# apple/ml-mdm

Hardware: AMD Instinct MI355X
Metric: denoise-steps/sec, whole job = N x optimizer steps/s at per-GPU batch 64 (train fwd+bwd+optimizer, cc12m_64x64 U-Net) (higher is better)
Workload: dtype bf16; 1 GPU; unet64 train step, per-GPU batch 64, global batch 64; global_batch=64, parallelism=dp1, settle_steps=15

## Files before the change

### include/mdm_hip_ext.h

```cpp
#ifndef MDM_HIP_EXT_H_
#define MDM_HIP_EXT_H_
#ifdef __cplusplus
extern "C" {
#endif

int mdm_attn_cross_bias(const void* qkv, const void* kvc, const float* mask, const float* bias, int bias_ld,
                        const void* base, int base_ld, void* out, int B, int L, int S, int H, int d, int dtype,
                        void* stream);

int mdm_freeu_plan(int N, int H, int W, int C1, int C2, int dtype, int structure, size_t* ws_bytes);
int mdm_freeu_stats(const void* h, const void* r, void* ws, size_t ws_bytes, int N, int H, int W, int C1, int C2,
                    int structure, int dtype, void* stream);
int mdm_freeu_apply(const void* h, const void* r, const void* ws, size_t ws_bytes, void* out, int N, int H, int W, int C1,
                    int C2, float b, float s, int structure, int dtype, void* stream);

int mdm_cfg_plan(int B, size_t chw, int rescale_on, size_t* ws_bytes);
int mdm_cfg_stats(const float* x_t, const float* pred, const float* pred_uncond, const float* gamma, const float* run_prev,
                  float* run_out, const float* run_gate, const float* w_gate, float momentum, int rescale_on, void* ws,
                  size_t ws_bytes, int B, size_t chw, int pred_type, void* stream);
int mdm_cfg_combine(const float* x_t, const float* pred, const float* pred_uncond, const float* gamma, const float* run,
                    const float* w_gate, const void* ws, size_t ws_bytes, float* out, float guidance, float eta,
                    float norm_threshold, float rescale, float image_scale, int B, size_t chw, int pred_type, void* stream);

int mdm_tiles_gather(const float* x, float* out, int B, int C, int H, int W, int h, int w, int sy, int sx, int reps,
                     void* stream);
int mdm_tiles_merge(const float* p, float* out, int R, int C, int H, int W, int h, int w, int sy, int sx, int blend,
                    void* stream);

int mdm_abs_quantile_plan(int B, size_t n, size_t* ws_bytes);
int mdm_abs_quantile(const float* x, void* ws, size_t ws_bytes, int B, size_t n, float q, float cmin, float cmax, float* thr,
                     float* stats, void* stream);

int mdm_t5_attn_fwd_lse(const void* qkv, const int* seq_start, const int* pos, const float* bias_table, void* out, float* lse,
                        int B, int T, int S, int max_len, int H, int d, int dtype, void* stream);
int mdm_t5_attn_bwd(const void* qkv, const void* out, const float* lse, const void* dout, const int* seq_start, const int* pos,
                    const float* bias_table, void* dqkv, int B, int T, int S, int max_len, int H, int d, int dtype,
                    void* stream);
int mdm_t5_gated_gelu_bwd(const void* u, const void* dy, void* du, int T, int F, int dtype, void* stream);
int mdm_t5_rms_bwd(const float* x, const float* ln_w, const void* dh, float* dx, void* dx_lo, int T, int D, float eps,
                   int dtype, void* stream);
int mdm_t5_final_rms_bwd(const float* x, const void* delta, const float* ln_w, const float* dout, const int* flat, float* dx,
                         void* dx_lo, int T, int D, float eps, int dtype, void* stream);
int mdm_t5_embed_rms_slots(const int* ids, const float* table, const int* slot_of_id, const float* learned, const float* ln_w,
                           float* x, void* h, int T, int D, int vocab, int n_ids, int P, float eps, int dtype, void* stream);
int mdm_t5_embed_bwd(const float* dx0, const int* slot_start, const int* tokens, float* dlearned, int P, int D, int n, int T,
                     void* stream);

int mdm_sampler_step_sa(const float* x_t, const float* pred, const float* pred_uncond, float guidance, const float* gamma,
                        const float* gamma_last, const float* gamma_h0, const float* gamma_h1, const float* gate,
                        const float* thr, const float* noise, const unsigned long long* rng_state, int rng_stream, float* h0,
                        float* h1, float* psum, float* x0_out, float* x_last_out, int B, size_t chw, int pred_type, int clip,
                        float image_scale, int max_predictor, int max_corrector, void* stream);

#ifdef __cplusplus
}
#endif
#endif
```

### ml-mdm_amd/csrc/gemm_conv.hip

```cpp
#include <stdio.h>
#include <stdlib.h>

#include <type_traits>
#include <utility>

#include "common.hpp"
#include "conv_args.hpp"

namespace mdm {



__device__ __forceinline__ void load4(const float* p, float (&o)[4]) {
  const f32x4 t = *reinterpret_cast<const f32x4*>(p);
  o[0] = t[0]; o[1] = t[1]; o[2] = t[2]; o[3] = t[3];
}
__device__ __forceinline__ void load4(const bf16* p, float (&o)[4]) {
  const bf16x4 t = *reinterpret_cast<const bf16x4*>(p);
  o[0] = (float)t[0]; o[1] = (float)t[1]; o[2] = (float)t[2]; o[3] = (float)t[3];
}

__device__ __attribute__((aligned(16))) uint4 g_zero_page[4] = {};


// ... 503 lines not shown
#pragma unroll
      for (int i = 0; i < MT; ++i) {
#pragma unroll
        for (int j = 0; j < NT; ++j) mma16(acc[i][j], b0[j], af[i]);
        load_frag<T>(af[i], As, wm * TM + i * 16 + l16, 1, quad);
      }
      __builtin_amdgcn_sched_group_barrier(0x100, NT, 0);
      sched_rows<NT, 0>(std::make_integer_sequence<int, MT>{});
      __builtin_amdgcn_sched_barrier(0);
      asm volatile("s_waitcnt vmcnt(%0)" ::"n"((NSTG - 2) * (AJ + BJ)) : "memory");
      __syncthreads();
      __builtin_amdgcn_sched_barrier(0);
      const char* An = smem + ((kt + 1) % NSTG) * STAGE;
      const char* Bn = An + A_BYTES;
      char* dst = smem + (kt % NSTG) * STAGE;
      MDM_TILE_STATE(kt + NSTG);
#pragma unroll
      for (int j = 0; j < NT; ++j) load_frag<T>(b0[j], Bn, wn * TN + j * 16 + l16, 0, quad);
#pragma unroll
      for (int i = 0; i < MT; ++i) {
#pragma unroll
        for (int j = 0; j < NT; ++j) mma16(acc[i][j], b1[j], af[i]);
#pragma unroll
        for (int d = 0; d < DMA_PER_ROW; ++d) { MDM_DMA_PIECE(dst, i * DMA_PER_ROW + d); }
        load_frag<T>(af[i], An, wm * TM + i * 16 + l16, 0, quad);
      }
      __builtin_amdgcn_sched_group_barrier(0x100, NT, 0);
      sched_rows<NT, DMA_PER_ROW>(std::make_integer_sequence<int, MT>{});
      __builtin_amdgcn_sched_barrier(0);
    }
    asm volatile("s_waitcnt vmcnt(0)" ::: "memory");
    __syncthreads();
    const int cur_m0 = m0, cur_n0 = n0;
    const int next = tile + G;
    if constexpr (SPLITK) {
      float* __restrict__ P = p.part + (size_t)split * p.M * p.Cout;
      if (next < tiles_total) {
        MDM_TILE_SETUP(next);
        MDM_TILE_PROLOGUE();
      }
#pragma unroll
      for (int i = 0; i < MT; ++i) {
        const int m = cur_m0 + wm * TM + i * 16 + l16;
        if (m >= p.M) continue;
#pragma unroll
        for (int j = 0; j < NT; ++j) {
          const int n = cur_n0 + wn * TN + j * 16 + quad * 4;
          if (n < p.Cout) *reinterpret_cast<f32x4*>(P + (size_t)m * p.Cout + n) = acc[i][j];
        }
      }
    } else {
      ConvArgs pe = p;
      if constexpr (GROUPED) { pe.bias = gr.bias[grp]; pe.y = gr.y[grp]; }
      auto prefetch_next = [&]() {
        if (next < tiles_total) {
          MDM_TILE_SETUP(next);
          MDM_TILE_PROLOGUE();
        }
      };
      conv_epilogue<T, BM, BN, WM, WN, NSTG * STAGE, decltype(prefetch_next)>(pe, acc, smem, cur_m0, cur_n0, prefetch_next);
    }
    if (next >= tiles_total) break;
    tile = next;
  }
#undef MDM_TILE_PROLOGUE
#undef MDM_TILE_SETUP
#undef MDM_DMA_PIECE
#undef MDM_TILE_STATE
#undef MDM_BLDS
#endif
}

struct WgradArgs {
  const void* x;
  const void* dy;
  float* slab;
  float* bslab;
  int N, H, W, Cin, Ho, Wo, Cout, stride;
  int M, K;
  int splits, mtiles_per_split;
  int groups;
  int bias_share;
  int skip_cout;
};

constexpr int WG_MAXG = 32;
constexpr int WG_BHDR = 64;
constexpr int WG_BSHARE = 4;
struct WgradGroup {
  const void* x[WG_MAXG];
  const void* dy[WG_MAXG];
  float* out[WG_MAXG];
  float* bout[WG_MAXG];
};

template <typename T, int MODE>
__global__ __launch_bounds__(256) void conv_wgrad_kernel(WgradArgs p) {
  constexpr int EPV = Tr<T>::EPV, BKM = Tr<T>::BK, KSTEPS = Tr<T>::KSTEPS;
  constexpr int BM = 128, BN = 128;
  constexpr int TM = 64, TN = 64, MT = 4, NT = 4;
  constexpr int A_BYTES = BM * 128, STAGE = 2 * A_BYTES;
  constexpr int CPR = 128 / EPV;
  constexpr int MB = BKM / EPV;
  constexpr int BLOCKS = CPR * MB;
  constexpr int NB = 2 * BLOCKS / 256;
  extern __shared__ __attribute__((aligned(16))) char smem[];

  const int tid = threadIdx.x, lane = tid & 63, wave = tid >> 6;
  const int wm = wave >> 1, wn = wave & 1;
  const int quad = lane >> 4, l16 = lane & 15;

  const int tiles_k = (p.K + BN - 1) / BN;
  const int tiles_n = (p.Cout + BM - 1) / BM;
  const int tiles = tiles_k * tiles_n;
  const int lid = xcd_remap(blockIdx.x, gridDim.x);
  const int split = lid / tiles;
  const int t = lid - split * tiles;
  const int n0 = (t / tiles_k) * BM, k0 = (t % tiles_k) * BN;

  const T* __restrict__ X = reinterpret_cast<const T*>(p.x);
  const T* __restrict__ DY = reinterpret_cast<const T*>(p.dy);

  int b_op[NB], b_cc[NB], b_mb[NB];
  int b_tap[NB], b_cin[NB];
  bool b_cvalid[NB];
#pragma unroll
  for (int i = 0; i < NB; ++i) {
    const int id = tid + 256 * i;
    b_op[i] = id / BLOCKS;
    const int r = id - b_op[i] * BLOCKS;
    b_mb[i] = r % MB;
    b_cc[i] = r / MB;
    if (b_op[i] == 0) {
      b_cvalid[i] = (n0 + b_cc[i] * EPV) < p.Cout;
      b_tap[i] = 0; b_cin[i] = 0;
    } else {
      const int k = k0 + b_cc[i] * EPV;
      b_cvalid[i] = k < p.K;
      if (MODE == MODE_1x1) { b_tap[i] = 0; b_cin[i] = k; }
      else { b_tap[i] = k / p.Cin; b_cin[i] = k - b_tap[i] * p.Cin; }
    }
  }

  Blk<T> blk[NB];
  const int mt_begin = split * p.mtiles_per_split;
  const int mt_total = (p.M + BKM - 1) / BKM;
  const int mt_end = min(mt_total, mt_begin + p.mtiles_per_split);

#define MDM_WG_LOAD(mt)                                                                                  \
  {                                                                                                      \
    _Pragma("unroll") for (int i = 0; i < NB; ++i) {                                                     \
      const bool is_a = b_op[i] == 0;                                                                    \
      const T* base = is_a ? DY : X;                                                                     \
      const int mbase = (mt) * BKM + b_mb[i] * EPV;                                                      \
      int pn = 0, poh = 0, pow_ = 0;                                                                     \
      if (MODE != MODE_1x1) {                                                                            \
        const int hw = p.Ho * p.Wo;                                                                      \
        pn = mbase / hw;                                                                                 \
        const int r = mbase - pn * hw;                                                                   \
        poh = r / p.Wo; pow_ = r - poh * p.Wo;                                                           \
      }                                                                                                  \
      const int kh = (b_tap[i] * 11) >> 5, kw = b_tap[i] - 3 * kh;                                       \
      const size_t a_col = (size_t)(n0 + b_cc[i] * EPV);                                                 \
      _Pragma("unroll") for (int e = 0; e < EPV; ++e) {                                                  \
        const int m = mbase + e;                                                                         \
        bool v = b_cvalid[i] && m < p.M;                                                                 \
// ... 543 lines not shown
    for (int c = 0; c < NT; ++c) fb[c] = smem_base + A_BYTES + r0 * ROWB + (((wn * NT + c) ^ fsw) << 5) + ((l16 & 3) << 3);
  }

  if (nt > 0) {
    {
      MDM_WG_TILE_STATE(0);
      MDM_WG_PIECE(smem, 0); MDM_WG_PIECE(smem, 1); MDM_WG_PIECE(smem, 2); MDM_WG_PIECE(smem, 3);
      MDM_WG_PIECE(smem, 4); MDM_WG_PIECE(smem, 5); MDM_WG_PIECE(smem, 6); MDM_WG_PIECE(smem, 7);
    }
    {
      MDM_WG_TILE_STATE(1);
      MDM_WG_PIECE(smem + STAGE, 0); MDM_WG_PIECE(smem + STAGE, 1); MDM_WG_PIECE(smem + STAGE, 2); MDM_WG_PIECE(smem + STAGE, 3);
      MDM_WG_PIECE(smem + STAGE, 4); MDM_WG_PIECE(smem + STAGE, 5); MDM_WG_PIECE(smem + STAGE, 6); MDM_WG_PIECE(smem + STAGE, 7);
    }
    asm volatile("s_waitcnt vmcnt(0)" ::: "memory");
    __syncthreads();
    u32x2 ra[MT][2], rb0[NT][2], rb1[NT][2];
#pragma unroll
    for (int c = 0; c < NT; ++c) MDM_TR2(rb0[c][0], rb0[c][1], fb[c], 0);
#pragma unroll
    for (int c = 0; c < MT; ++c) MDM_TR2(ra[c][0], ra[c][1], fa[c], 0);
    __builtin_amdgcn_sched_barrier(0);

#define MDM_WG_ITER(BIAS)                                                                                   \
    {                                                                                                       \
      const unsigned so = (unsigned)((it & 1) * STAGE), sn = (unsigned)(((it + 1) & 1) * STAGE);            \
                                                                     \
      _Pragma("unroll") for (int c = 0; c < NT; ++c) { const unsigned ad = fb[c] + so; MDM_TR2(rb1[c][0], rb1[c][1], ad, KS1); } \
      Frag<T> bq[NT];                                                                                       \
      _Pragma("unroll") for (int i = 0; i < MT; ++i) {                                                      \
        if (i == 0) {                                                                                       \
          asm volatile("s_waitcnt lgkmcnt(%8)"                                                              \
                       : "+v"(rb0[0][0]), "+v"(rb0[0][1]), "+v"(rb0[1][0]), "+v"(rb0[1][1]), "+v"(rb0[2][0]), \
                         "+v"(rb0[2][1]), "+v"(rb0[3][0]), "+v"(rb0[3][1])                                  \
                       : "n"(WAITN) : "memory");                                                            \
          _Pragma("unroll") for (int j = 0; j < NT; ++j) bq[j] = frag_of(rb0[j][0], rb0[j][1]);             \
        }                                                                                                   \
        asm volatile("s_waitcnt lgkmcnt(%2)" : "+v"(ra[i][0]), "+v"(ra[i][1]) : "n"(WAITN) : "memory");     \
        const Frag<T> aq = frag_of(ra[i][0], ra[i][1]);                                                     \
        _Pragma("unroll") for (int j = 0; j < NT; ++j) mma16(acc[i][j], bq[j], aq);                         \
        if (BIAS && i / BR == wn_s) bsum[i % BR] = frag_sum_guarded(aq, bsum[i % BR]);                      \
        { const unsigned ad = fa[i] + so; MDM_TR2(ra[i][0], ra[i][1], ad, KS1); }                           \
        __builtin_amdgcn_sched_barrier(0);                                                                  \
      }                                                                                                     \
                                        \
      asm volatile("s_waitcnt vmcnt(0) lgkmcnt(0)" ::: "memory");                                           \
      __builtin_amdgcn_s_barrier();                                                                         \
      __builtin_amdgcn_sched_barrier(0);                                                                    \
              \
      MDM_WG_TILE_STATE(it + 2);                                                                            \
      char* const dst = smem + so;                                                                          \
      _Pragma("unroll") for (int c = 0; c < NT; ++c) { const unsigned ad = fb[c] + sn; MDM_TR2(rb0[c][0], rb0[c][1], ad, 0); } \
      _Pragma("unroll") for (int j = 0; j < NT; ++j) bq[j] = frag_of(rb1[j][0], rb1[j][1]);                 \
      _Pragma("unroll") for (int i = 0; i < MT; ++i) {                                                      \
        const Frag<T> aq = frag_of(ra[i][0], ra[i][1]);                                                     \
        _Pragma("unroll") for (int j = 0; j < NT; ++j) mma16(acc[i][j], bq[j], aq);                         \
        if (BIAS && i / BR == wn_s) bsum[i % BR] = frag_sum_guarded(aq, bsum[i % BR]);                      \
        if (MT == 8) { MDM_WG_PIECE_RT(dst, i) } else { MDM_WG_PIECE_RT(dst, 2 * i) MDM_WG_PIECE_RT(dst, 2 * i + 1) } \
        { const unsigned ad = fa[i] + sn; MDM_TR2(ra[i][0], ra[i][1], ad, 0); }                             \
        __builtin_amdgcn_sched_barrier(0);                                                                  \
      }                                                                                                     \
    }
#define MDM_WG_PIECE_RT(stage, q)                                                                           \
    switch (q) {                                                                                            \
      case 0: MDM_WG_PIECE(stage, 0) break; case 1: MDM_WG_PIECE(stage, 1) break;                           \
      case 2: MDM_WG_PIECE(stage, 2) break; case 3: MDM_WG_PIECE(stage, 3) break;                           \
      case 4: MDM_WG_PIECE(stage, 4) break; case 5: MDM_WG_PIECE(stage, 5) break;                           \
      case 6: MDM_WG_PIECE(stage, 6) break; default: MDM_WG_PIECE(stage, 7) break;                          \
    }
    int it = 0;
    float bsum[BR];
    for (; it < bias_b0; ++it) MDM_WG_ITER(false)
#pragma unroll
    for (int i = 0; i < BR; ++i) bsum[i] = 0.f;
    for (; it < bias_b1; ++it) MDM_WG_ITER(true)
    if (bias_blk) {
#pragma unroll
      for (int r = 0; r < BR; ++r) {
        float v = bsum[r];
        v += __shfl_xor(v, 16, 64);
        v += __shfl_xor(v, 32, 64);
        const int n = n0 + wm * TM + (wn * BR + r) * 16 + l16;
        if (quad == 0 && n < p.Cout) {
          if (p.groups > 0) gr.bout[grp][n] += v;
          else p.bslab[((size_t)split * bias_share + kt_rel) * p.Cout + n] = v;
        }
      }
    }
    for (; it < nt; ++it) MDM_WG_ITER(false)
    asm volatile("s_waitcnt vmcnt(0) lgkmcnt(0)" ::: "memory");
#undef MDM_WG_PIECE_RT
#undef MDM_WG_ITER
  } else if (bias_blk && p.groups == 0 && quad == 0) {
#pragma unroll
    for (int r = 0; r < BR; ++r) {
      const int n = n0 + wm * TM + (wn * BR + r) * 16 + l16;
      if (n < p.Cout) p.bslab[((size_t)split * bias_share + kt_rel) * p.Cout + n] = 0.f;
    }
  }
#undef MDM_WG_PIECE
#undef MDM_WG_TILE_STATE
#undef MDM_BLDS

  if (bias_blk && p.groups == 0 && split == 0 && kt_rel == 0 && n0 == 0 && tid == 0)
    reinterpret_cast<int*>(p.bslab - WG_BHDR)[0] = bias_share;
  const bool direct = p.groups > 0;
  float* __restrict__ S = direct ? gr.out[grp] : p.slab + (size_t)split * p.Cout * p.K;
  const bool vec_ok = (p.K & 3) == 0;
  if (!direct) {
#pragma unroll
    for (int i = 0; i < MT; ++i) {
      const int n = n0 + wm * TM + i * 16 + l16;
      if (n >= p.Cout) continue;
#pragma unroll
      for (int j = 0; j < NT; ++j) {
        const int k = k0 + wn * TN + j * 16 + quad * 4;
        if (k >= p.K) continue;
        float* o = S + (size_t)n * p.K + k;
        if (vec_ok) {
          *reinterpret_cast<f32x4*>(o) = acc[i][j];
        } else {
#pragma unroll
          for (int e = 0; e < 4; ++e) if (k + e < p.K) o[e] = acc[i][j][e];
        }
      }
    }
  } else if (vec_ok && n0 + BM <= p.Cout && k0 + BN <= p.K) {
    float* const o0 = S + (size_t)(n0 + wm * TM + l16) * p.K + k0 + wn * TN + quad * 4;
    f32x4 old[2][NT];
#pragma unroll
    for (int j = 0; j < NT; ++j) old[0][j] = *reinterpret_cast<const f32x4*>(o0 + j * 16);
#pragma unroll
    for (int i = 0; i < MT; ++i) {
      if (i + 1 < MT) {
#pragma unroll
        for (int j = 0; j < NT; ++j) old[(i + 1) & 1][j] = *reinterpret_cast<const f32x4*>(o0 + (size_t)(i + 1) * 16 * p.K + j * 16);
      }
#pragma unroll
      for (int j = 0; j < NT; ++j) *reinterpret_cast<f32x4*>(o0 + (size_t)i * 16 * p.K + j * 16) = old[i & 1][j] + acc[i][j];
    }
  } else {
#pragma unroll
    for (int i = 0; i < MT; ++i) {
      const int n = n0 + wm * TM + i * 16 + l16;
      if (n >= p.Cout) continue;
#pragma unroll
      for (int j = 0; j < NT; ++j) {
        const int k = k0 + wn * TN + j * 16 + quad * 4;
        if (k >= p.K) continue;
        float* o = S + (size_t)n * p.K + k;
#pragma unroll
        for (int e = 0; e < 4; ++e) if (k + e < p.K) o[e] += acc[i][j][e];
      }
    }
  }
#endif
}
#undef MDM_TR2

template <int NT>
__device__ __forceinline__ void wgrad_bias_reduce(const float* __restrict__ bslab, float* __restrict__ dbias, int splits,
                                                  int Cout, int accumulate, int blk, float* lds) {
  constexpr int G = NT / 32;
  const int tid = threadIdx.x, c = tid & 31, g = tid >> 5;
  const int rows = splits * reinterpret_cast<const int*>(bslab - WG_BHDR)[0];
  const int o = blk * 32 + c;
  float s0 = 0.f, s1 = 0.f, s2 = 0.f, s3 = 0.f;
  if (o < Cout) {
    const float* src = bslab + o;
    int r = g;
    for (; r + 3 * G < rows; r += 4 * G) {
      s0 += src[(size_t)r * Cout];
      s1 += src[(size_t)(r + G) * Cout];
      s2 += src[(size_t)(r + 2 * G) * Cout];
      s3 += src[(size_t)(r + 3 * G) * Cout];
    }
    for (; r < rows; r += G) s0 += src[(size_t)r * Cout];
  }
  lds[tid] = (s0 + s1) + (s2 + s3);
  __syncthreads();
  if (g == 0 && o < Cout) {
    float s = lds[c];
#pragma unroll
    for (int q = 1; q < G; ++q) s += lds[q * 32 + c];
    dbias[o] = accumulate ? dbias[o] + s : s;
  }
}

__global__ __launch_bounds__(192) void wgrad_reduce_kernel(const float* __restrict__ slab, float* __restrict__ dw,
                                                           const float* __restrict__ bslab, float* __restrict__ dbias,
                                                           int splits, int Cout, int Cin, int taps, int accumulate,
                                                           int bblocks) {
// ... 1122 lines not shown
  a.mtiles_per_split = (mt_total + a.splits - 1) / a.splits;
  float* const bias_ws = ws + (size_t)a.splits * Cout * a.K;
  a.bslab = (want_bias && dtype == DT_BF16) ? bias_ws + WG_BHDR : nullptr;
  const int te = wgrad_tile(a.M, Cout, a.K, dtype);
  const int tiles = ((Cout + te - 1) / te) * ((a.K + te - 1) / te);
  {
    const int kt = skip_cout > 0 ? Cin / te : (a.K + te - 1) / te;
    a.bias_share = kt < WG_BSHARE ? (kt < 1 ? 1 : kt) : WG_BSHARE;
  }
  hipStream_t st = reinterpret_cast<hipStream_t>(stream);
  if (wgrad_direct_slabs(a.M, Cout, a.K, dtype) && wgrad_direct_ok(a, ksize)) {
    return launch_wgrad_direct<64, 9, 8>(a, st);
  }
  constexpr int smem = 4 * 128 * 128, smem_big = 4 * 64 * 512;
  ensure_dynamic_lds(conv_wgrad_kernel<float, MODE_1x1>, smem);
  ensure_dynamic_lds(conv_wgrad_kernel<float, MODE_3x3>, smem);
  ensure_dynamic_lds(conv_wgrad_tr_kernel<MODE_1x1, 0>, smem);
  ensure_dynamic_lds(conv_wgrad_tr_kernel<MODE_3x3, 0>, smem);
  ensure_dynamic_lds(conv_wgrad_tr_kernel<MODE_1x1, 1>, smem_big);
  ensure_dynamic_lds(conv_wgrad_tr_kernel<MODE_3x3, 1>, smem_big);
  ensure_dynamic_lds(conv_wgrad_bl_kernel<MODE_1x1, 0>, smem);
  ensure_dynamic_lds(conv_wgrad_bl_kernel<MODE_3x3, 0>, smem);
  ensure_dynamic_lds(conv_wgrad_bl_kernel<MODE_1x1, 1>, smem_big);
  ensure_dynamic_lds(conv_wgrad_bl_kernel<MODE_3x3, 1>, smem_big);
  dim3 grid(tiles * a.splits);
  const int mode = ksize == 1 ? MODE_1x1 : MODE_3x3;
  if (dtype == DT_F32) MDM_NOTE_KERNEL("conv_wgrad_kernel<float, %d>", mode);
  else if (wgrad_bl_ok(a, ksize)) MDM_NOTE_KERNEL("conv_wgrad_bl_kernel<%d, %d>", mode, te == 256 ? 1 : 0);
  else MDM_NOTE_KERNEL("conv_wgrad_tr_kernel<%d, %d>", mode, te == 256 ? 1 : 0);
  if (dtype == DT_F32) {
    if (ksize == 1) hipLaunchKernelGGL((conv_wgrad_kernel<float, MODE_1x1>), grid, dim3(256), smem, st, a);
    else hipLaunchKernelGGL((conv_wgrad_kernel<float, MODE_3x3>), grid, dim3(256), smem, st, a);
  } else if (wgrad_bl_ok(a, ksize)) {
    if (te == 256) {
      if (ksize == 1) hipLaunchKernelGGL((conv_wgrad_bl_kernel<MODE_1x1, 1>), grid, dim3(512), smem_big, st, a, WgradGroup{});
      else hipLaunchKernelGGL((conv_wgrad_bl_kernel<MODE_3x3, 1>), grid, dim3(512), smem_big, st, a, WgradGroup{});
    } else {
      if (ksize == 1) hipLaunchKernelGGL((conv_wgrad_bl_kernel<MODE_1x1, 0>), grid, dim3(256), smem, st, a, WgradGroup{});
      else hipLaunchKernelGGL((conv_wgrad_bl_kernel<MODE_3x3, 0>), grid, dim3(256), smem, st, a, WgradGroup{});
    }
  } else if (te == 256) {
    if (ksize == 1) hipLaunchKernelGGL((conv_wgrad_tr_kernel<MODE_1x1, 1>), grid, dim3(512), smem_big, st, a);
    else hipLaunchKernelGGL((conv_wgrad_tr_kernel<MODE_3x3, 1>), grid, dim3(512), smem_big, st, a);
  } else {
    if (ksize == 1) hipLaunchKernelGGL((conv_wgrad_tr_kernel<MODE_1x1, 0>), grid, dim3(256), smem, st, a);
    else hipLaunchKernelGGL((conv_wgrad_tr_kernel<MODE_3x3, 0>), grid, dim3(256), smem, st, a);
  }
  MDM_LAUNCH_STATUS();
}

extern "C" int mdm_conv_wgrad(const void* x, const void* dy, int want_bias, float* ws, int N, int H, int W, int Cin,
                              int Ho, int Wo, int Cout, int ksize, int stride, int dtype, void* stream) {
  return conv_wgrad_impl(x, dy, want_bias, ws, N, H, W, Cin, Ho, Wo, Cout, ksize, stride, dtype, 0, stream);
}

extern "C" int mdm_conv_wgrad_blocked(const void* x, const void* dyb, int want_bias, float* ws, int N, int H, int W, int Cin,
                                      int Cout, int dtype, void* stream) {
  MDM_CHECK_ARG(dtype == DT_BF16 && Cin % 256 == 0 && Cout % 256 == 0);
  MDM_CHECK_ARG((H & (H - 1)) == 0 && (W & (W - 1)) == 0);
  return conv_wgrad_impl(x, dyb, want_bias, ws, N, H, W, Cin, H, W, 4 * Cout, 3, 1, dtype, Cout, stream);
}

static int wgrad_group_tile(int M, int Cout, int K, int groups) {
  if (groups < 2 || groups > WG_MAXG || M < 4096) return 0;
  if (const int forced = wgrad_forced_tile(Cout, K, DT_BF16)) return forced;
  const long t256 = (long)((Cout + 255) / 256) * ((K + 255) / 256) * groups;
  const long t128 = (long)((Cout + 127) / 128) * ((K + 127) / 128) * groups;
  const int cus = device_cus();
  if (Cout >= 192 && K >= 192) {
    const double eff = (double)t256 / (double)(((t256 + cus - 1) / cus) * cus);
    if (t256 >= (long)(0.7 * cus) && eff >= 0.7) return 256;
  }
  const double eff = (double)t128 / (double)(((t128 + 2 * cus - 1) / (2 * cus)) * 2 * cus);
  if (t128 >= (long)(1.4 * cus) && eff >= 0.7) return 128;
  return 0;
}

extern "C" int mdm_conv_wgrad_group_plan(int M, int Cout, int K, int dtype, int groups, int* tile_out) {
  MDM_CHECK_ARG(tile_out);
  *tile_out = dtype == DT_BF16 ? wgrad_group_tile(M, Cout, K, groups) : 0;
  return 0;
}

extern "C" int mdm_conv_wgrad_grouped(const void* const* x, const void* const* dy, float* const* dw,
                                      float* const* dbias, int groups, int M, int Cin, int Cout, int dtype,
                                      void* stream) {
  MDM_CHECK_ARG(x && dy && dw && groups >= 1 && groups <= WG_MAXG);
  MDM_CHECK_ARG(dtype == DT_BF16 && Cin % 8 == 0 && Cout % 8 == 0 && M > 0);
  WgradArgs a = {};
  a.N = M; a.H = 1; a.W = 1; a.Cin = Cin; a.Ho = 1; a.Wo = 1; a.Cout = Cout; a.stride = 1;
  a.M = M; a.K = Cin; a.splits = 1; a.groups = groups;
  a.mtiles_per_split = (M + 63) / 64;
  MDM_CHECK_ARG(wgrad_bl_ok(a, 1));
  WgradGroup gr = {};
  for (int g = 0; g < groups; ++g) {
    MDM_CHECK_ARG(x[g] && dy[g] && dw[g]);
    gr.x[g] = x[g]; gr.dy[g] = dy[g]; gr.out[g] = dw[g]; gr.bout[g] = dbias ? dbias[g] : nullptr;
  }
  int te = wgrad_group_tile(M, Cout, Cin, groups);
  if (!te) te = wgrad_forced_tile(Cout, Cin, DT_BF16);
  if (!te) te = (Cout >= 192 && Cin >= 192) ? 256 : 128;
  const int tiles = ((Cout + te - 1) / te) * ((Cin + te - 1) / te);
  hipStream_t st = reinterpret_cast<hipStream_t>(stream);
  constexpr int smem = 4 * 128 * 128, smem_big = 4 * 64 * 512;
  if (te == 256) {
    ensure_dynamic_lds(conv_wgrad_bl_kernel<MODE_1x1, 1>, smem_big);
    hipLaunchKernelGGL((conv_wgrad_bl_kernel<MODE_1x1, 1>), dim3(tiles * groups), dim3(512), smem_big, st, a, gr);
  } else {
    ensure_dynamic_lds(conv_wgrad_bl_kernel<MODE_1x1, 0>, smem);
    hipLaunchKernelGGL((conv_wgrad_bl_kernel<MODE_1x1, 0>), dim3(tiles * groups), dim3(256), smem, st, a, gr);
  }
  MDM_NOTE_KERNEL("conv_wgrad_bl_kernel<%d, %d>", MODE_1x1, te == 256 ? 1 : 0);
  MDM_LAUNCH_STATUS();
}

extern "C" int mdm_conv_wgrad_reduce(const float* ws, float* dw_oihw, float* dbias, const void* dy, int M, int Cin,
                                     int Cout, int ksize, int accumulate, int dtype, void* stream) {
  MDM_CHECK_ARG(ws && dw_oihw && (ksize == 1 || ksize == 3));
  const int K = ksize * ksize * Cin;
  int splits; size_t wsb;
  int rc = mdm_conv_wgrad_plan(M, Cout, K, dtype, &splits, &wsb);
  if (rc) return rc;
  hipStream_t st = reinterpret_cast<hipStream_t>(stream);
  float* const bias_ws = const_cast<float*>(ws) + (size_t)splits * Cout * K;
  const float* bslab = (dbias && dtype == DT_BF16) ? bias_ws + WG_BHDR : nullptr;
  const int bblocks = bslab ? (Cout + 31) / 32 : 0;
  if (ksize == 1) {
    const size_t total = (size_t)Cout * Cin;
    const int wblocks = (int)((total / 4 + 255) / 256 > 2048 ? 2048 : (total / 4 + 255) / 256);
    hipLaunchKernelGGL(wgrad_reduce_flat_kernel, dim3(wblocks + bblocks), dim3(256), 0, st, ws, dw_oihw, bslab, dbias,
                       splits, Cout, total, accumulate, wblocks, bblocks);
  } else {
    const int wblocks = Cout * ((Cin + 63) / 64);
    hipLaunchKernelGGL(wgrad_reduce_kernel, dim3(wblocks + bblocks), dim3(192), 0, st, ws, dw_oihw, bslab, dbias,
                       splits, Cout, Cin, ksize * ksize, accumulate, bblocks);
  }
  if (dbias && !bslab) {
    MDM_CHECK_ARG(dy);
    return mdm_colsum(dy, dbias, bias_ws, M, Cout, accumulate, dtype, stream);
  }
  MDM_LAUNCH_STATUS();
}

extern "C" int mdm_pack_weight(const float* w_oihw, void* w_fwd, void* w_dgrad, int Cout, int Cin, int ksize,
                               int Cin_pad, int Cout_pad, int kblock_fwd, int kblock_dgrad, int dtype,
                               void* stream) {
  MDM_CHECK_ARG(w_oihw && w_fwd);
  MDM_CHECK_ARG(ksize == 1 || ksize == 3);
  MDM_CHECK_ARG(Cin_pad >= Cin && Cout_pad >= Cout);
  MDM_CHECK_ARG(kblock_fwd == 0 || (ksize == 3 && Cin_pad % kblock_fwd == 0));
  MDM_CHECK_ARG(kblock_dgrad == 0 || (ksize == 3 && Cout_pad % kblock_dgrad == 0));
  const int taps = ksize * ksize;
  const size_t total = (size_t)Cout * taps * Cin_pad + (w_dgrad ? (size_t)Cin * taps * Cout_pad : 0);
  const int nb = (int)((total + 255) / 256 > 8192 ? 8192 : (total + 255) / 256);
  hipStream_t st = reinterpret_cast<hipStream_t>(stream);
  if (Cin_pad == Cin && Cout_pad == Cout && Cin % 32 == 0 && Cout % 32 == 0) {
    dim3 grid(Cin / 32, Cout / 32);
#define MDM_PACK_TILED(TT, TAPS)                                                                               \
  hipLaunchKernelGGL((pack_weight_tiled_kernel<TT, TAPS>), grid, dim3(256), 0, st, w_oihw, (TT*)w_fwd, (TT*)w_dgrad, \
                     Cout, Cin, kblock_fwd, kblock_dgrad)
    if (dtype == DT_F32) { if (taps == 9) MDM_PACK_TILED(float, 9); else MDM_PACK_TILED(float, 1); }
    else if (dtype == DT_BF16) { if (taps == 9) MDM_PACK_TILED(bf16, 9); else MDM_PACK_TILED(bf16, 1); }
    else MDM_CHECK_ARG(false);
#undef MDM_PACK_TILED
    MDM_LAUNCH_STATUS();
  }
  if (dtype == DT_F32)
    hipLaunchKernelGGL(pack_weight_kernel<float>, dim3(nb), dim3(256), 0, st, w_oihw, (float*)w_fwd, (float*)w_dgrad, Cout, Cin, taps, Cin_pad, Cout_pad, kblock_fwd, kblock_dgrad);
  else if (dtype == DT_BF16)
    hipLaunchKernelGGL(pack_weight_kernel<bf16>, dim3(nb), dim3(256), 0, st, w_oihw, (bf16*)w_fwd, (bf16*)w_dgrad, Cout, Cin, taps, Cin_pad, Cout_pad, kblock_fwd, kblock_dgrad);
  else MDM_CHECK_ARG(false);
  MDM_LAUNCH_STATUS();
}

extern "C" int mdm_pack_weights_multi(const void* table, int n, int total_blocks, int dtype, void* stream) {
  MDM_CHECK_ARG(table && n > 0 && total_blocks > 0);
  static_assert(sizeof(PackDesc) == 48, "descriptor layout is part of the ABI");
  hipStream_t st = reinterpret_cast<hipStream_t>(stream);
  if (dtype == DT_F32) hipLaunchKernelGGL(pack_weights_multi_kernel<float>, dim3(total_blocks), dim3(256), 0, st, (const PackDesc*)table, n);
  else if (dtype == DT_BF16) hipLaunchKernelGGL(pack_weights_multi_kernel<bf16>, dim3(total_blocks), dim3(256), 0, st, (const PackDesc*)table, n);
  else MDM_CHECK_ARG(false);
  MDM_LAUNCH_STATUS();
}

static inline int colsum_slabs(int M, int C, int epv) {
  const int groups = (C + 8 * epv - 1) / (8 * epv);
  int slabs = (1024 + groups - 1) / groups;
  const int max_slabs = (M + 63) / 64;
  if (slabs > max_slabs) slabs = max_slabs;
  if (slabs > 64) slabs = 64;
  if (slabs < 1) slabs = 1;
  return slabs;
}

extern "C" int mdm_colsum_plan(int M, int C, int* nblocks, size_t* ws_bytes) {
  MDM_CHECK_ARG(nblocks && ws_bytes);
// ... 24 lines not shown
```

### ml-mdm_amd/csrc/norm.hip

```cpp
#include <stdlib.h>

#include "common.hpp"

namespace mdm {

template <int N> struct GnInt { static constexpr int value = N; };

template <int ACT>
__device__ __forceinline__ float gn_affine_act(float a, float x, float b) {
  const float z = a * x + b;
  return ACT ? silu_f(z) : z;
}


template <typename T>
__global__ __launch_bounds__(256) void gn_partial_kernel(const T* __restrict__ x, float* __restrict__ part,
                                                         int HW, int C, int slabs, int pix_per_slab) {
  constexpr int EPV = Tr<T>::EPV;
  __shared__ float red[256 * 16];
  const int n = blockIdx.x / slabs, slab = blockIdx.x - n * slabs;
  const int tid = threadIdx.x;
  const int nchunks = C / EPV;
  const int p_begin = slab * pix_per_slab, p_end = min(HW, p_begin + pix_per_slab);
  const T* xn = x + (size_t)n * HW * C;
// ... 1006 lines not shown
#define MDM_GN_REAPPLY(TT, ACT, DROP)                                                                                \
  hipLaunchKernelGGL((gn_reapply_kernel<TT, ACT, DROP>), grid, dim3(256), 0, st, (const TT*)x, coef, (TT*)y, HW, C, lanes, \
                     ppb, thresh, scale, seed, offset)
#define MDM_GN_REAPPLY_T(TT)                                                                                         \
  if (p > 0.f) { if (act) MDM_GN_REAPPLY(TT, 1, true); else MDM_GN_REAPPLY(TT, 0, true); }                           \
  else { if (act) MDM_GN_REAPPLY(TT, 1, false); else MDM_GN_REAPPLY(TT, 0, false); }
  if (dtype == DT_F32) { MDM_GN_REAPPLY_T(float) } else { MDM_GN_REAPPLY_T(bf16) }
#undef MDM_GN_REAPPLY_T
#undef MDM_GN_REAPPLY
  MDM_LAUNCH_STATUS();
}

extern "C" int mdm_gn_bwd(const void* dy, const void* x, const float* gamma, const float* beta, const void* film,
                          const float* stats, const float* coef, const void* dres, const void* dres2, void* dx,
                          float* dgamma, float* dbeta, void* dfilm, float* ws, int N, int HW, int C, int G, int act,
                          int accumulate, int dtype, void* stream) {
  MDM_CHECK_ARG(dy && x && gamma && beta && stats && coef && dx && dgamma && dbeta && ws);
  MDM_CHECK_ARG(dtype == DT_F32 || dtype == DT_BF16);
  MDM_CHECK_ARG((film == nullptr) == (dfilm == nullptr));
  if (!dres && dres2) { dres = dres2; dres2 = nullptr; }
  const int epv = dtype == DT_F32 ? 4 : 8;
  MDM_CHECK_ARG(C % epv == 0 && C % G == 0 && C <= 2048 && G <= 256);
  hipStream_t st = reinterpret_cast<hipStream_t>(stream);
  MDM_CHECK_ARG(accumulate >= 0 && accumulate <= 2);
  const int pstride = accumulate == 2 ? C : 0;
  if (!accumulate) {
    if (hipMemsetAsync(dgamma, 0, (size_t)C * sizeof(float), st) != hipSuccess ||
        hipMemsetAsync(dbeta, 0, (size_t)C * sizeof(float), st) != hipSuccess) {
      mdm_set_error(__FILE__, __LINE__, "hipMemsetAsync(dgamma / dbeta)");
      return (int)hipGetLastError();
    }
  }
  if (const GnFusedCfg f = gn_fused_cfg(HW, C, G, dtype, true); f.cb) {
    const dim3 grid(N, C / f.cb);
    const int cb = f.cb;
#define MDM_GN_FUSED_BWD_L(TT, ACT, NI_, NT_, LPR_)                                                                 \
    hipLaunchKernelGGL((gn_fused_bwd_kernel<TT, ACT, NI_, NT_, LPR_>), grid, dim3(NT_), 0, st, (const TT*)dy, (const TT*)x, gamma, beta, (const TT*)film, stats, coef, (TT*)dx, (TT*)dfilm, dgamma, dbeta, (const TT*)dres, (const TT*)dres2, HW, C, G, cb, pstride)
#define MDM_GN_FUSED_BWD(TT, ACT, LPR_)                                                                             \
    if (f.nthr == 512 && f.ni == 4) MDM_GN_FUSED_BWD_L(TT, ACT, 4, 512, LPR_);                                     \
    else if (f.nthr == 512) MDM_GN_FUSED_BWD_L(TT, ACT, 16, 512, LPR_);                                            \
    else MDM_GN_FUSED_BWD_L(TT, ACT, 4, 1024, LPR_)
    if (dtype == DT_F32) { if (act) { MDM_GN_FUSED_BWD(float, 1, 16); } else { MDM_GN_FUSED_BWD(float, 0, 16); } }
    else { if (act) { MDM_GN_FUSED_BWD(bf16, 1, 8); } else { MDM_GN_FUSED_BWD(bf16, 0, 8); } }
#undef MDM_GN_FUSED_BWD
#undef MDM_GN_FUSED_BWD_L
    MDM_LAUNCH_STATUS();
  }
  const int cb = gn_slice(C, G, epv);
  MDM_CHECK_ARG(cb > 0);
  const size_t esize = dtype == DT_F32 ? 4 : 2;
  int nchunk = 1;
  while (nchunk < 8 && N % (nchunk * 2) == 0 && N / (nchunk * 2) >= 4 &&
         2 * (size_t)N * HW * C * esize / nchunk > g_gn_chunk_bytes)
    nchunk *= 2;
  if ((size_t)(N / nchunk) * gn_slabs(N / nchunk, HW) > (size_t)N * gn_slabs(N, HW)) nchunk = 1;
  const int nc = N / nchunk;
  const int slabs = gn_slabs(nc, HW);
  const int pps = (HW + slabs - 1) / slabs;
  const int sp = gn_pix_splits(nc, HW, C / cb);
  const int ppb = (HW + sp - 1) / sp;
  const dim3 agrid(sp, C / cb, nc);
#define MDM_GN_BWD(TT, ACT)                                                                                          \
  for (int ch = 0; ch < nchunk; ++ch) {                                                                              \
    const size_t n0 = (size_t)ch * nc, t0 = n0 * HW * C;                                                             \
    const TT* film_ = film ? (const TT*)film + n0 * 2 * C : nullptr;                                                 \
    TT* dfilm_ = dfilm ? (TT*)dfilm + n0 * 2 * C : nullptr;                                                          \
    const TT* dres_ = dres ? (const TT*)dres + t0 : nullptr;                                                         \
    const TT* dres2_ = dres2 ? (const TT*)dres2 + t0 : nullptr;                                                      \
    hipLaunchKernelGGL((gn_bwd_partial_kernel<TT, ACT>), dim3(nc * slabs), dim3(256), 0, st, (const TT*)dy + t0,     \
                       (const TT*)x + t0, coef + n0 * C * 2, ws, HW, C, slabs, pps);                                 \
    hipLaunchKernelGGL((gn_bwd_apply_kernel<TT, ACT>), agrid, dim3(256), 0, st, (const TT*)dy + t0, (const TT*)x + t0, ws, \
                       stats + n0 * G * 2, coef + n0 * C * 2, gamma, beta, film_, dres_, dres2_, (TT*)dx + t0, dfilm_, \
                       dgamma + n0 * pstride, dbeta + n0 * pstride, HW, C, G, cb, slabs, ppb, pstride);              \
  }
  if (dtype == DT_F32) { if (act) { MDM_GN_BWD(float, 1) } else { MDM_GN_BWD(float, 0) } }
  else { if (act) { MDM_GN_BWD(bf16, 1) } else { MDM_GN_BWD(bf16, 0) } }
#undef MDM_GN_BWD
  MDM_LAUNCH_STATUS();
}

struct GnParamDesc {
  const float* pg; const float* pb;
  float* dgamma; float* dbeta;
  int N, C, first_block, pad_;
};

__global__ __launch_bounds__(256) void gn_param_reduce_multi_kernel(const GnParamDesc* __restrict__ table, int n) {
  __shared__ float red[2][4][64];
  const int lb = (int)blockIdx.x >> 2, sub = (int)blockIdx.x & 3;
  int lo = 0, hi = n - 1;
  while (lo < hi) {
    const int mid = (lo + hi + 1) >> 1;
    if (table[mid].first_block <= lb) lo = mid; else hi = mid - 1;
  }
  const GnParamDesc d = table[lo];
  const int cl = (int)threadIdx.x & 63, q = (int)threadIdx.x >> 6;
  const int c = (lb - d.first_block) * 256 + sub * 64 + cl;
  float a = 0.f, b = 0.f;
  if (c < d.C) {
    int s_ = q;
    for (; s_ + 12 < d.N; s_ += 16) {
      const float a0 = d.pg[(size_t)s_ * d.C + c], a1 = d.pg[(size_t)(s_ + 4) * d.C + c];
      const float a2 = d.pg[(size_t)(s_ + 8) * d.C + c], a3 = d.pg[(size_t)(s_ + 12) * d.C + c];
      const float b0 = d.pb[(size_t)s_ * d.C + c], b1 = d.pb[(size_t)(s_ + 4) * d.C + c];
      const float b2 = d.pb[(size_t)(s_ + 8) * d.C + c], b3 = d.pb[(size_t)(s_ + 12) * d.C + c];
      a += (a0 + a1) + (a2 + a3);
      b += (b0 + b1) + (b2 + b3);
    }
    for (; s_ < d.N; s_ += 4) { a += d.pg[(size_t)s_ * d.C + c]; b += d.pb[(size_t)s_ * d.C + c]; }
  }
  red[0][q][cl] = a; red[1][q][cl] = b;
  __syncthreads();
  if (q == 0 && c < d.C) {
    d.dgamma[c] += (red[0][0][cl] + red[0][1][cl]) + (red[0][2][cl] + red[0][3][cl]);
    d.dbeta[c] += (red[1][0][cl] + red[1][1][cl]) + (red[1][2][cl] + red[1][3][cl]);
  }
}

extern "C" int mdm_gn_param_reduce_multi(const void* table, int n, int total_blocks, void* stream) {
  MDM_CHECK_ARG(table && n > 0 && total_blocks > 0);
  static_assert(sizeof(GnParamDesc) == 48, "descriptor layout is part of the ABI");
  hipLaunchKernelGGL(gn_param_reduce_multi_kernel, dim3(4 * total_blocks), dim3(256), 0, reinterpret_cast<hipStream_t>(stream),
                     (const GnParamDesc*)table, n);
  MDM_LAUNCH_STATUS();
}

extern "C" int mdm_ln_fwd(const void* x, const float* gamma, const float* beta, void* y, float* stats, int R, int D,
                          float eps, int dtype, void* stream) {
  MDM_CHECK_ARG(x && gamma && beta && y && stats && R > 0 && D > 0);
  hipStream_t st = reinterpret_cast<hipStream_t>(stream);
  if (dtype == DT_F32) hipLaunchKernelGGL(ln_fwd_kernel<float>, dim3(R), dim3(256), 0, st, (const float*)x, gamma, beta, (float*)y, stats, D, eps);
  else if (dtype == DT_BF16) hipLaunchKernelGGL(ln_fwd_kernel<bf16>, dim3(R), dim3(256), 0, st, (const bf16*)x, gamma, beta, (bf16*)y, stats, D, eps);
  else MDM_CHECK_ARG(false);
  MDM_LAUNCH_STATUS();
}

extern "C" int mdm_ln_bwd(const void* dy, const void* x, const float* gamma, const float* stats, void* dx,
                          float* dgamma, float* dbeta, float* ws, int R, int D, int accumulate, int dtype,
                          void* stream) {
  MDM_CHECK_ARG(dy && x && gamma && stats && dx && dgamma && dbeta && ws);
  hipStream_t st = reinterpret_cast<hipStream_t>(stream);
  const int rpb = 64, nsl = (R + rpb - 1) / rpb;
  if (dtype == DT_F32) {
    hipLaunchKernelGGL(ln_bwd_kernel<float>, dim3(R), dim3(256), 0, st, (const float*)dy, (const float*)x, gamma, stats, (float*)dx, D);
    hipLaunchKernelGGL(ln_bwd_param_partial_kernel<float>, dim3((D + 255) / 256, nsl), dim3(256), 0, st, (const float*)dy, (const float*)x, stats, ws, R, D, rpb);
  } else if (dtype == DT_BF16) {
    hipLaunchKernelGGL(ln_bwd_kernel<bf16>, dim3(R), dim3(256), 0, st, (const bf16*)dy, (const bf16*)x, gamma, stats, (bf16*)dx, D);
    hipLaunchKernelGGL(ln_bwd_param_partial_kernel<bf16>, dim3((D + 255) / 256, nsl), dim3(256), 0, st, (const bf16*)dy, (const bf16*)x, stats, ws, R, D, rpb);
  } else MDM_CHECK_ARG(false);
  hipLaunchKernelGGL(ln_bwd_param_final_kernel, dim3((D + 255) / 256), dim3(256), 0, st, ws, dgamma, dbeta, nsl, D, accumulate);
  MDM_LAUNCH_STATUS();
}

extern "C" int mdm_ln_multi_fwd(const void* x, const float* const* gamma, const float* const* beta, void* const* y, int L,
                                float* stats, int R, int D, float eps, int dtype, void* stream) {
  MDM_CHECK_ARG(x && gamma && beta && y && stats && L >= 1 && L <= LN_MAXL && R > 0 && D > 0);
  MDM_CHECK_ARG(dtype == DT_F32 ? (D % 4 == 0 && D <= 256 * 4 * LN_NCK) : (D % 8 == 0 && D <= 256 * 8 * LN_NCK));
  LnGroup g = {};
  for (int l = 0; l < L; ++l) { MDM_CHECK_ARG(gamma[l] && beta[l] && y[l]); g.gamma[l] = gamma[l]; g.beta[l] = beta[l]; g.y[l] = y[l]; }
  hipStream_t st = reinterpret_cast<hipStream_t>(stream);
  if (dtype == DT_F32) hipLaunchKernelGGL(ln_multi_fwd_kernel<float>, dim3(R), dim3(256), 0, st, (const float*)x, g, L, stats, D, eps);
  else if (dtype == DT_BF16) hipLaunchKernelGGL(ln_multi_fwd_kernel<bf16>, dim3(R), dim3(256), 0, st, (const bf16*)x, g, L, stats, D, eps);
  else MDM_CHECK_ARG(false);
  MDM_LAUNCH_STATUS();
}

extern "C" int mdm_ln_multi_bwd(const void* const* dy, const void* x, const float* const* gamma, const float* stats,
                                void* dx, float* const* dgamma, float* const* dbeta, int L, int R, int D, int accumulate,
                                int dtype, void* stream) {
  MDM_CHECK_ARG(dy && x && gamma && stats && dx && dgamma && dbeta && L >= 1 && L <= LN_MAXL && R > 0 && D > 0 && D <= 4096);
  MDM_CHECK_ARG(D % (dtype == DT_F32 ? 4 : 8) == 0);
  LnGroup g = {};
  hipStream_t st = reinterpret_cast<hipStream_t>(stream);
  for (int l = 0; l < L; ++l) {
    MDM_CHECK_ARG(dy[l] && gamma[l] && dgamma[l] && dbeta[l]);
    g.y[l] = const_cast<void*>(dy[l]); g.gamma[l] = gamma[l]; g.dgamma[l] = dgamma[l]; g.dbeta[l] = dbeta[l];
    if (!accumulate) {
      (void)hipMemsetAsync(dgamma[l], 0, (size_t)D * sizeof(float), st);
      (void)hipMemsetAsync(dbeta[l], 0, (size_t)D * sizeof(float), st);
    }
  }
  const int rpb = 64, nsl = (R + rpb - 1) / rpb;
  if (dtype == DT_F32) {
    hipLaunchKernelGGL(ln_multi_bwd_kernel<float>, dim3(R), dim3(256), 0, st, g, L, (const float*)x, stats, (float*)dx, D);
    hipLaunchKernelGGL(ln_multi_param_kernel<float>, dim3((D + 255) / 256, nsl, L), dim3(256), 0, st, g, (const float*)x, stats, R, D, rpb);
  } else if (dtype == DT_BF16) {
    hipLaunchKernelGGL(ln_multi_bwd_kernel<bf16>, dim3(R), dim3(256), 0, st, g, L, (const bf16*)x, stats, (bf16*)dx, D);
    hipLaunchKernelGGL(ln_multi_param_kernel<bf16>, dim3((D + 255) / 256, nsl, L), dim3(256), 0, st, g, (const bf16*)x, stats, R, D, rpb);
  } else MDM_CHECK_ARG(false);
  MDM_LAUNCH_STATUS();
}
```

### ml-mdm_amd/csrc/optim.hip

```cpp
#include "common.hpp"

namespace mdm {

__global__ __launch_bounds__(256) void sumsq_partial_kernel(const float* __restrict__ g, float* __restrict__ part,
                                                            size_t n4) {
  __shared__ float sh[4];
  float s = 0.f;
  const f32x4* g4 = reinterpret_cast<const f32x4*>(g);
  for (size_t i = (size_t)blockIdx.x * 256 + threadIdx.x; i < n4; i += (size_t)gridDim.x * 256) {
    const f32x4 v = g4[i];
    s += v[0] * v[0] + v[1] * v[1] + v[2] * v[2] + v[3] * v[3];
  }
  s = wave_sum(s);
  if ((threadIdx.x & 63) == 0) sh[threadIdx.x >> 6] = s;
  __syncthreads();
  if (threadIdx.x == 0) part[blockIdx.x] = sh[0] + sh[1] + sh[2] + sh[3];
}

__global__ __launch_bounds__(256) void sumsq_final_kernel(const float* __restrict__ part, int nparts,
                                                          const float* __restrict__ g, size_t n, size_t tail_from,
                                                          float* __restrict__ out, int* __restrict__ step_counter) {
  __shared__ float sh[4];
  float s = 0.f;
  for (int i = threadIdx.x; i < nparts; i += 256) s += part[i];
  for (size_t i = tail_from + threadIdx.x; i < n; i += 256) s += g[i] * g[i];
  s = wave_sum(s);
  if ((threadIdx.x & 63) == 0) sh[threadIdx.x >> 6] = s;
  __syncthreads();
  if (threadIdx.x == 0) {
    const float q = sh[0] + sh[1] + sh[2] + sh[3];
    out[0] = q;
    if (step_counter && q == q && q <= 3.0e38f) step_counter[0] += 1;
  }
}

struct AdamArgs {
  float* p; float* g; float* m; float* v; float* ema;
  const float* gnorm_sq;
  const int* step_dev;
  size_t n;
  float lr, beta1, beta2, eps, wd, bc1, bc2, clip, ema_decay;
  int zero_grad;
};

__device__ __forceinline__ void adam_one(float& p, float& g, float& m, float& v, float& e, const AdamArgs& a, float gs,
                                         bool has_ema) {
  const float gr = g * gs;
  p *= (1.f - a.lr * a.wd);
  m = a.beta1 * m + (1.f - a.beta1) * gr;
  v = a.beta2 * v + (1.f - a.beta2) * gr * gr;
  const float denom = sqrtf(v) / sqrtf(a.bc2) + a.eps;
  p -= (a.lr / a.bc1) * (m / denom);
  if (has_ema) e = e * a.ema_decay + p * (1.f - a.ema_decay);
  if (a.zero_grad) g = 0.f;
}

__global__ __launch_bounds__(256) void adamw_ema_kernel(AdamArgs a) {
  if (a.step_dev) {
    const float st = (float)a.step_dev[0];
    a.bc1 = 1.f - powf(a.beta1, st);
    a.bc2 = 1.f - powf(a.beta2, st);
  }
  float gs = 1.f;
  bool poisoned = false;
  if (a.gnorm_sq) {
    const float q = a.gnorm_sq[0];
    poisoned = !(q == q) || q > 3.0e38f;
    const float nrm = sqrtf(q);
    gs = fminf(a.clip / (nrm + 1e-6f), 1.f);
  }
  const bool has_ema = a.ema != nullptr;
  const size_t n4 = a.n / 4;
  f32x4* p4 = reinterpret_cast<f32x4*>(a.p);
  f32x4* g4 = reinterpret_cast<f32x4*>(a.g);
  if (poisoned) {
    if (a.zero_grad) {
      for (size_t i = (size_t)blockIdx.x * 256 + threadIdx.x; i < n4; i += (size_t)gridDim.x * 256) g4[i] = f32x4{0.f, 0.f, 0.f, 0.f};
      if (blockIdx.x == 0) for (size_t i = n4 * 4 + threadIdx.x; i < a.n; i += 256) a.g[i] = 0.f;
    }
    return;
  }
  f32x4* m4 = reinterpret_cast<f32x4*>(a.m);
  f32x4* v4 = reinterpret_cast<f32x4*>(a.v);
  f32x4* e4 = reinterpret_cast<f32x4*>(a.ema);
  for (size_t i = (size_t)blockIdx.x * 256 + threadIdx.x; i < n4; i += (size_t)gridDim.x * 256) {
    f32x4 p = p4[i], g = g4[i], m = m4[i], v = v4[i];
    f32x4 e = has_ema ? e4[i] : f32x4{0.f, 0.f, 0.f, 0.f};
#pragma unroll
    for (int k = 0; k < 4; ++k) {
      float pp = p[k], gg = g[k], mm = m[k], vv = v[k], ee = e[k];
      adam_one(pp, gg, mm, vv, ee, a, gs, has_ema);
      p[k] = pp; g[k] = gg; m[k] = mm; v[k] = vv; e[k] = ee;
    }
    p4[i] = p; m4[i] = m; v4[i] = v;
    if (has_ema) e4[i] = e;
    if (a.zero_grad) g4[i] = g;
  }
  if (blockIdx.x == 0) {
    for (size_t i = n4 * 4 + threadIdx.x; i < a.n; i += 256) {
      float e = has_ema ? a.ema[i] : 0.f;
      adam_one(a.p[i], a.g[i], a.m[i], a.v[i], e, a, gs, has_ema);
      if (has_ema) a.ema[i] = e;
    }
  }
}

}

using namespace mdm;

extern "C" int mdm_sumsq(const float* g, float* out, float* ws, size_t n, int* step_counter, void* stream) {
  MDM_CHECK_ARG(g && out && ws);
  MDM_CHECK_ARG(((size_t)g & 15) == 0);
  hipStream_t st = reinterpret_cast<hipStream_t>(stream);
  const size_t n4 = n / 4;
  int nb = (int)((n4 + 255) / 256 > 1024 ? 1024 : (n4 + 255) / 256);
  if (nb < 1) nb = 1;
  hipLaunchKernelGGL(sumsq_partial_kernel, dim3(nb), dim3(256), 0, st, g, ws, n4);
  hipLaunchKernelGGL(sumsq_final_kernel, dim3(1), dim3(256), 0, st, ws, nb, g, n, n4 * 4, out, step_counter);
  MDM_LAUNCH_STATUS();
}

extern "C" int mdm_adamw_ema_step(float* p, float* g, float* m, float* v, float* ema, const float* gnorm_sq, size_t n,
                                  float lr, float beta1, float beta2, float eps, float weight_decay, int step,
                                  const int* step_dev, float clip, float ema_decay, int zero_grad, void* stream) {
  MDM_CHECK_ARG(p && g && m && v && (step >= 1 || step_dev));
  MDM_CHECK_ARG((((size_t)p | (size_t)g | (size_t)m | (size_t)v | (size_t)ema) & 15) == 0);
  AdamArgs a;
  a.p = p; a.g = g; a.m = m; a.v = v; a.ema = ema; a.gnorm_sq = gnorm_sq; a.n = n;
  a.lr = lr; a.beta1 = beta1; a.beta2 = beta2; a.eps = eps; a.wd = weight_decay;
  a.step_dev = step_dev;
  a.bc1 = 1.f - powf(beta1, (float)(step >= 1 ? step : 1));
  a.bc2 = 1.f - powf(beta2, (float)(step >= 1 ? step : 1));
  a.clip = clip; a.ema_decay = ema_decay; a.zero_grad = zero_grad;
  hipStream_t st = reinterpret_cast<hipStream_t>(stream);
  const size_t n4 = n / 4;
  int nb = (int)((n4 + 255) / 256 > 8192 ? 8192 : (n4 + 255) / 256);
  if (nb < 1) nb = 1;
  hipLaunchKernelGGL(adamw_ema_kernel, dim3(nb), dim3(256), 0, st, a);
  MDM_LAUNCH_STATUS();
}
```

### ml-mdm_amd/mdm_hip/distributed.py

```python
import os
from datetime import timedelta

import torch
import torch.distributed as dist


def get_rank() -> int:
    return dist.get_rank() if dist.is_available() and dist.is_initialized() else 0


def get_world_size() -> int:
    return dist.get_world_size() if dist.is_available() and dist.is_initialized() else 1


def get_local_rank() -> int:
    return int(os.environ.get("LOCAL_RANK", "0"))


def print0(*a, **k):
    if get_rank() == 0:
        print(*a, **k)


def init_distributed_singlenode(timeout: int = 0, backend: str = None):
    world = int(os.environ.get("WORLD_SIZE", "1"))
    if world == 1 or "MASTER_ADDR" not in os.environ:
        return get_local_rank(), int(os.environ.get("RANK", "0")), 1
    rank, local = int(os.environ["RANK"]), get_local_rank()
    if backend is None:
        backend = "nccl" if torch.cuda.is_available() else "gloo"
    kw = {"timeout": timedelta(seconds=timeout)} if timeout else {}
    if backend == "nccl":
        torch.cuda.set_device(local)
    dist.init_process_group(backend=backend, init_method="env://", world_size=world, rank=rank, **kw)
    barrier(local)
    return local, rank, world


def barrier(local_rank: int = None):
    if dist.get_backend() == "nccl":
        dist.barrier(device_ids=[torch.cuda.current_device() if local_rank is None else local_rank])
    else:
        dist.barrier()


class GradReducer:

    def __init__(self, params, bucket_mb: float = 256.0, wire_dtype="auto", group=None, tail_mb: float = 8.0,
                 world_override: int = None, force_collectives: bool = False, head_mb: float = 64.0,
                 record_timeline: bool = False, late_params=None):
        self.params = [p for p in params if p.requires_grad]
        self.group = group
        self.nranks = dist.get_world_size(group) if dist.is_initialized() else 1
        if world_override is not None:
            self.nranks = int(world_override)
        self.world = self.nranks if not (force_collectives and self.nranks == 1 and dist.is_initialized()) else 2
        self._wire_auto = False
        if isinstance(wire_dtype, str):
            if wire_dtype != "auto":
                raise ValueError("wire_dtype: a torch dtype, None (fp32) or 'auto'")
            wire_dtype = None
        self.wire_dtype = wire_dtype
        self._wire = {}
        self._comm = None
        self._avg_ok = None
        self.record_timeline = bool(record_timeline)
        self._timeline = []
        self._t0 = None
        dev = self.params[0].device
        total = sum(p.numel() for p in self.params)
        self.flat = torch.zeros(total, dtype=torch.float32, device=dev)
        order = list(reversed(self.params))
        late = {id(p) for p in (late_params or [])}
        if late:
            order = [p for p in order if id(p) not in late] + [p for p in order if id(p) in late]
        self.order = order
        cap = max(1, int(bucket_mb * (1 << 20) / 4))
        tail = min(int(tail_mb * (1 << 20) / 4), cap)
        head = max(1, min(int(head_mb * (1 << 20) / 4), cap)) if head_mb else cap
        tail_from, acc = len(order), 0
        for i in range(len(order) - 1, -1, -1):
            acc += order[i].numel()
            if acc > tail:
                break
            tail_from = i
        self.buckets = []
        self._bucket_of = {}
        off = b_start = 0
        for i, p in enumerate(order):
            if i == tail_from and off > b_start:
                self.buckets.append((b_start, off))
                b_start = off
            n = p.numel()
            p.grad = self.flat[off:off + n].view_as(p)
            self._bucket_of[p] = len(self.buckets)
            off += n
            if off - b_start >= (head if not self.buckets else cap):
                self.buckets.append((b_start, off))
                b_start = off
        if off > b_start:
            self.buckets.append((b_start, off))
        self._slots = {p.data_ptr(): (p, p.grad) for p in self.params}
        self._grad_ptrs = [(p, p.grad.data_ptr()) for p in self.params]
        self._need = [0] * len(self.buckets)
        for p in order:
            self._need[self._bucket_of[p]] += 1
        self._pending = list(self._need)
        self._fired = {}
        self._deferred = set()
        self._streams = [set() for _ in self.buckets]
        self._work = []
        self._enabled = True
        if self.world > 1:
            for p in self.params:
                p.register_post_accumulate_grad_hook(self._hook)

    def slot(self, p):
        ent = self._slots.get(p.data_ptr())
        return ent[1] if ent is not None and ent[0].shape == p.shape else None

    def ready(self, p):
        if self.world > 1:
            self._count(self._slots[p.data_ptr()][0])

    def defer(self, p):
        if self.world > 1:
            self._deferred.add(id(self._slots[p.data_ptr()][0]))

    def rebind(self):
        self._slots = {p.data_ptr(): (p, p.grad) for p in self.params}

    def _hook(self, p):
        if id(p) in self._deferred:
            return
        self._count(p)

    def note_autocast(self, bf16: bool):
        return None

    def _comm_stream(self):
        if self._comm is None:
            self._comm = torch.cuda.Stream(device=self.flat.device)
        return self._comm

    def _post_stream(self):
        if getattr(self, "_post", None) is None:
            self._post = torch.cuda.Stream(device=self.flat.device)
        return self._post

    def _count(self, p):
        if not self._enabled:
            return
        b = self._bucket_of[p]
        if id(p) in self._fired:
            return
        self._fired[id(p)] = 1
        if p.is_cuda:
            self._streams[b].add(torch.cuda.current_stream())
        self._pending[b] -= 1
        if self._pending[b] == 0:
            self._launch(b)

    def _launch(self, b):
        s, e = self.buckets[b]
        buf = self.flat[s:e]
        if not buf.is_cuda:
            buf.div_(self.nranks)
            if self.wire_dtype is not None and self.wire_dtype != torch.float32:
                wire = buf.to(self.wire_dtype)
                h = dist.all_reduce(wire, op=dist.ReduceOp.SUM, group=self.group, async_op=True)
                self._work.append((h, buf, wire, None))
            else:
                h = dist.all_reduce(buf, op=dist.ReduceOp.SUM, group=self.group, async_op=True)
                self._work.append((h, None, None, None))
            return
        comm = self._comm_stream()
        for st in self._streams[b]:
            ev = torch.cuda.Event()
            ev.record(st)
            comm.wait_event(ev)
        self._streams[b] = set()
        post = self._post_stream()
        with torch.cuda.stream(comm):
            ev0 = None
            if self.record_timeline:
                if self._t0 is None:
                    self._t0 = torch.cuda.Event(enable_timing=True)
                    self._t0.record(comm)
                ev0 = torch.cuda.Event(enable_timing=True)
                ev0.record(comm)
            scale = 1.0 / self.nranks
            if self.wire_dtype is not None and self.wire_dtype != torch.float32:
                wire = self._wire.get(b)
                if wire is None:
                    wire = self._wire[b] = torch.empty(e - s, dtype=self.wire_dtype, device=buf.device)
                if self.nranks > 1:
                    torch.mul(buf, scale, out=wire)
                else:
                    wire.copy_(buf)
                h = dist.all_reduce(wire, op=dist.ReduceOp.SUM, group=self.group, async_op=True)
                nbytes = wire.numel() * wire.element_size()
            else:
                wire = None
                if self._avg_ok is None:
                    self._avg_ok = dist.get_backend(self.group) == "nccl" and hasattr(dist.ReduceOp, "AVG")
                if self._avg_ok and self.nranks > 1:
                    h = dist.all_reduce(buf, op=dist.ReduceOp.AVG, group=self.group, async_op=True)
                else:
                    if self.nranks > 1:
                        buf.mul_(scale)
                    h = dist.all_reduce(buf, op=dist.ReduceOp.SUM, group=self.group, async_op=True)
                nbytes = buf.numel() * 4
        with torch.cuda.stream(post):
            h.wait()
            if wire is not None:
                buf.copy_(wire)
            done = None
            if ev0 is not None:
                done = torch.cuda.Event(enable_timing=True)
                done.record(post)
                self._timeline.append([b, nbytes, ev0, done])
        self._work.append((h, None, None, ev0))

    def no_sync(self):
        reducer = self

        class _Ctx:
            def __enter__(self):
                reducer._enabled = False

            def __exit__(self, *a):
                reducer._enabled = True

        return _Ctx()

    def check_bound(self):
        for p, ptr in self._grad_ptrs:
            if p.grad is None or p.grad.data_ptr() != ptr:
                raise RuntimeError("a parameter's .grad no longer points into the GradReducer arena (zero_grad(set_to_none=True)?); "
                                   "use GradReducer.zero_grad()")

    def finish(self):
        self.check_bound()
        if self.world > 1 and self._enabled:
            if self._pending == self._need and not self._work:
                self._deferred = set()
                return
            missing = [b for b, n in enumerate(self._pending) if n != 0]
            if missing:
                lost = [(i, tuple(p.shape), self._fired.get(id(p), 0)) for i, p in enumerate(self.params) if self._fired.get(id(p), 0) != 1]
                raise RuntimeError("buckets %s did not receive all their gradients; parameters (index, shape) that "
                                   "did not report exactly once (index, shape, count): %s" % (missing, lost[:12]))
            if self._comm is not None and self.flat.is_cuda:
                torch.cuda.current_stream().wait_stream(self._post_stream())
            else:
                for h, buf, wire, _ in self._work:
                    h.wait()
                    if wire is not None:
                        buf.copy_(wire)
            self._work = []
            if self.record_timeline:
                self._last_timeline, self._last_t0 = self._timeline, self._t0
                self._timeline, self._t0 = [], None
            self._pending = list(self._need)
            self._fired = {}
        self._deferred = set()

    def mark(self, what):
        if self.record_timeline and self.flat.is_cuda and self.world > 1:
            ev = torch.cuda.Event(enable_timing=True)
            ev.record()
            setattr(self, "_" + what, ev)

    def backward_window_ms(self):
        b0, b1, t0 = getattr(self, "_bw0", None), getattr(self, "_bw1", None), getattr(self, "_last_t0", None)
        if b0 is None or b1 is None or t0 is None:
            return None
        torch.cuda.synchronize()
        return b0.elapsed_time(t0), b0.elapsed_time(b1)

    def timeline(self):
        tl, t0 = getattr(self, "_last_timeline", None), getattr(self, "_last_t0", None)
        if not tl or t0 is None:
            return []
        torch.cuda.synchronize()
        return [(b, nb, t0.elapsed_time(e0), t0.elapsed_time(e1) if e1 is not None else float("nan")) for b, nb, e0, e1 in tl]

    def zero_grad(self):
        self.flat.zero_()

    def broadcast_parameters(self, src: int = 0):
        if self.nranks == 1:
            return
        with torch.no_grad():
            chunk, acc = [], 0
            for p in self.params:
                chunk.append(p)
                acc += p.numel()
                if acc * 4 >= (256 << 20):
                    self._bcast(chunk, src)
                    chunk, acc = [], 0
            if chunk:
                self._bcast(chunk, src)

    def _bcast(self, ps, src):
        flat = torch.cat([p.detach().reshape(-1) for p in ps])
        dist.broadcast(flat, src, group=self.group)
        off = 0
        for p in ps:
            p.copy_(flat[off:off + p.numel()].view_as(p))
            off += p.numel()


class DataParallel(torch.nn.Module):

    _IGNORED = {"output_device", "dim", "broadcast_buffers", "process_group", "bucket_cap_mb", "check_reduction",
                "gradient_as_bucket_view", "init_sync", "device_mesh", "mixed_precision", "delay_all_reduce_named_params",
                "param_to_hook_all_reduce"}
    _UNSUPPORTED = {"find_unused_parameters", "static_graph"}

    def __init__(self, module, device_ids=None, bucket_mb: float = 256.0, wire_dtype="auto", tail_mb: float = 8.0,
                 force_collectives: bool = False, head_mb: float = 64.0, record_timeline: bool = False, **ddp_kwargs):
        super().__init__()
        for k, v in ddp_kwargs.items():
            if k in self._UNSUPPORTED:
                if v:
                    raise ValueError("mdm_hip.distributed.DataParallel does not implement %s=True: every parameter of the "
                                     "vision model must receive a gradient in every synchronised backward" % k)
            elif k not in self._IGNORED:
                raise TypeError("DataParallel got an unexpected keyword argument %r" % k)
        if ddp_kwargs.get("process_group") is not None:
            raise ValueError("process_group: pass the group to GradReducer directly (the default group is used here)")
        self.module = module
        net = getattr(module, "vision_model", module)
        late = net.late_gradient_parameters() if hasattr(net, "late_gradient_parameters") else None
        self.reducer = GradReducer(list(net.parameters()), bucket_mb=bucket_mb, wire_dtype=wire_dtype, tail_mb=tail_mb,
                                   force_collectives=force_collectives, head_mb=head_mb, record_timeline=record_timeline,
                                   late_params=late)
        self.reducer.broadcast_parameters(0)

    def forward(self, *args, **kwargs):
        return self.module(*args, **kwargs)

    def no_sync(self):
        return self.reducer.no_sync()
```

### ml-mdm_amd/mdm_hip/ops.py

```python
import ctypes
import weakref

import torch

from . import _lib
from . import tiling as _tiling

F32, BF16, F32_SPLIT, F32_SPLIT_W = 0, 1, 2, 3

_fp32_split = False
_weight_planes_on = True


class fp32_split:

    def __init__(self, enabled: bool = True):
        global _fp32_split
        self._prev = _fp32_split
        _fp32_split = bool(enabled)

    def __enter__(self):
        return self

    def __exit__(self, *a):
        global _fp32_split
        _fp32_split = self._prev


def fp32_split_enabled() -> bool:
    return _fp32_split


def _dt_mm(t: torch.Tensor) -> int:
    d = _dt(t)
    return F32_SPLIT if (d == F32 and _fp32_split) else d


def _dt(t: torch.Tensor) -> int:
    if t.dtype == torch.float32:
        return F32
    if t.dtype == torch.bfloat16:
        return BF16
    raise _lib.MdmHipError("unsupported activation dtype %s" % t.dtype)


def _epv(t: torch.Tensor) -> int:
    return 4 if t.dtype == torch.float32 else 8


def _p(t):
    return None if t is None else t.data_ptr()


_raw_stream = getattr(torch._C, "_cuda_getCurrentRawStream", None)
_raw_device = getattr(torch._C, "_cuda_getDevice", None)


def _stream():
    if _raw_stream is not None and _raw_device is not None:
        return _raw_stream(_raw_device())
    return torch.cuda.current_stream().cuda_stream


_stream_objs = {}


def _current_stream_obj():
    raw = _stream()
    st = _stream_objs.get(raw)
    if st is None:
        if len(_stream_objs) > 64:
            _stream_objs.clear()
        st = _stream_objs[raw] = torch.cuda.current_stream()
    return st


def _require_gpu(t: torch.Tensor):
    if not t.is_cuda:
        raise _lib.MdmHipError(
            "mdm_hip ops run only on an MI355X (got a %s tensor); there is no CPU fallback" % t.device
        )


def _f32_ws(nbytes: int, device):
    return torch.empty((max(int(nbytes), 4) + 3) // 4, dtype=torch.float32, device=device)


def _c(t):
    return t if t is None or t.is_contiguous() else t.contiguous()


_wcache = {}
_pack_epoch = 0


def invalidate_packed_weights():
    global _pack_epoch
    _pack_epoch += 1


_grad_sink = None


def set_grad_sink(sink):
    global _grad_sink
    if _grad_sink is not None and sink is not _grad_sink:
        flush_wgrad_queue()
    _grad_sink = sink


def _slot(param):
    if _grad_sink is None or param is None:
        return None
    return _grad_sink.slot(param)


def _sink_defer(param):
    f = getattr(_grad_sink, "defer", None)
    if f is not None and param is not None:
        f(param)


_side_stream = None
_async_wgrad = False


def enable_async_wgrad(flag: bool):
    global _async_wgrad
    _async_wgrad = bool(flag)


def side_stream():
    global _side_stream
    if _side_stream is None:
        _side_stream = torch.cuda.Stream()
    return _side_stream


_side_keep = []


def join_side_stream():
    if _side_stream is not None:
        torch.cuda.current_stream().wait_stream(_side_stream)
    _side_keep.clear()


def _off_critical_path(tensors, fn):
    if not (_async_wgrad and _grad_sink is not None):
        return fn()
    side = side_stream()
    if _raw_stream is None:
        side.wait_stream(torch.cuda.current_stream())
        with torch.cuda.stream(side):
            fn()
            done = torch.cuda.Event()
            done.record(side)
    else:
        cur = _current_stream_obj()
        side.wait_stream(cur)
        torch.cuda.set_stream(side)
        try:
            fn()
            done = torch.cuda.Event()
            done.record(side)
        finally:
            torch.cuda.set_stream(cur)
    live = [t for t in tensors if t is not None]
    _side_keep.append((done, live))
    if len(_side_keep) >= 64:
        _side_keep[:] = [e for e in _side_keep if not e[0].query()]


_defer_wgrad = False
_wgrad_queue = {}
_WG_MAX = 32


def enable_deferred_wgrad(flag: bool, max_group: int = 32):
    global _defer_wgrad, _WG_MAX
    flush_wgrad_queue()
    _defer_wgrad = bool(flag)
    _WG_MAX = max(1, min(32, int(max_group)))


def wgrad_grouped(xs, dys, dws, dbs=None):
    G = len(xs)
    M, cin = xs[0].shape
    cout = dys[0].shape[1]
    for t in list(xs) + list(dys):
        _require_gpu(t)
    xs, dys = [_c(t) for t in xs], [_c(t) for t in dys]
    arr = lambda vals: (ctypes.c_void_p * G)(*vals)
    _lib.check(_lib.lib().mdm_conv_wgrad_grouped(arr([_p(t) for t in xs]), arr([_p(t) for t in dys]), arr([_p(t) for t in dws]),
                                                 arr([_p(t) for t in dbs]) if dbs is not None else None, G, M, cin, cout,
                                                 _dt(xs[0]), _stream()), "mdm_conv_wgrad_grouped")


def _queue_wgrad(x, dy, weight, bias, slot, bslot, M, cin, cout):
    key = (M, cin, cout, x.device.index)
    q = _wgrad_queue.setdefault(key, [])
    q.append((x, dy, weight, bias, slot, bslot))
    _sink_defer(weight)
    if bslot is not None:
        _sink_defer(bias)
    if len(q) == _WG_MAX:
        _flush_key(key)


def _flush_key(key):
    q = _wgrad_queue.pop(key, None)
    if not q:
        return
    M, cin, cout, _ = key
    L = _lib.lib()
    tile = ctypes.c_int(0)
    _lib.check(L.mdm_conv_wgrad_group_plan(M, cout, cin, BF16, len(q), ctypes.byref(tile)), "mdm_conv_wgrad_group_plan")
    tensors = [t for e in q for t in (e[0], e[1])]
    if tile.value and all((e[5] is not None) == (q[0][5] is not None) for e in q):
        G = len(q)
        arr = lambda vals: (ctypes.c_void_p * G)(*vals)
        xs, dys, dws = arr([_p(e[0]) for e in q]), arr([_p(e[1]) for e in q]), arr([_p(e[4]) for e in q])
        dbs = arr([_p(e[5]) for e in q]) if q[0][5] is not None else None

        def go():
            _prof_wrap("conv_wgrad grouped x%d M=%d N=%d K=%d" % (G, M, cout, cin), 2.0 * G * M * cout * cin, lambda: _lib.check(
                L.mdm_conv_wgrad_grouped(xs, dys, dws, dbs, G, M, cin, cout, BF16, _stream()), "mdm_conv_wgrad_grouped"))
            for e in q:
                _grad_sink.ready(e[2])
                if e[5] is not None:
                    _grad_sink.ready(e[3])
    else:
        def go():
            for x, dy, w, b, slot, bslot in q:
                _wgrad_launch(x, dy, M, 1, 1, cin, 1, 1, cout, 1, 1, out=slot, dbias=bslot)
                _grad_sink.ready(w)
                if bslot is not None:
                    _grad_sink.ready(b)

    _off_critical_path(tensors, go)


def flush_wgrad_queue():
    for key in list(_wgrad_queue):
        _flush_key(key)
    flush_gn_params()


_gn_pending = []
_gn_pool = {}
_gn_tables = {}


def _gn_rows(N, C, device):
    ent = _gn_pool.get(device.index)
    need = 2 * N * C
    if ent is None or ent[1] + need > ent[0].numel():
        size = max(need, 0 if ent is None else 2 * ent[0].numel(), 16 << 20)
        ent = _gn_pool[device.index] = [torch.empty(size, dtype=torch.float32, device=device), 0]
    off = ent[1]
    ent[1] = off + need
    return ent[0][off:off + N * C], ent[0][off + N * C:off + need]


def flush_gn_params():
    if not _gn_pending:
        return
    dev = _gn_pending[0][0].device
    key = tuple((e[0].data_ptr(), e[1].data_ptr(), e[2].data_ptr(), e[3].data_ptr(), e[4], e[5]) for e in _gn_pending)
    ent = _gn_tables.get(key)
    if ent is None:
        import numpy as np
        rec = np.zeros(len(key), dtype=[("pg", "<u8"), ("pb", "<u8"), ("dg", "<u8"), ("db", "<u8"), ("N", "<i4"),
                                         ("C", "<i4"), ("first", "<i4"), ("pad", "<i4")])
        blocks = 0
        for i, (pg, pb, dg, db, N, C) in enumerate(key):
            rec[i] = (pg, pb, dg, db, N, C, blocks, 0)
            blocks += (C + 255) // 256
        table = torch.from_numpy(rec.view(np.uint8).copy()).to(dev)
        if len(_gn_tables) > 64:
            _gn_tables.clear()
        ent = _gn_tables[key] = (table, blocks)
    table, blocks = ent
    _lib.check(_lib.lib().mdm_gn_param_reduce_multi(_p(table), len(key), blocks, _stream()), "mdm_gn_param_reduce_multi")
    for e in _gn_pending:
        _grad_sink.ready(e[6])
        _grad_sink.ready(e[7])
    _gn_pending.clear()
    for ent in _gn_pool.values():
        ent[1] = 0


class _FlushPointFn(torch.autograd.Function):

    @staticmethod
    def forward(ctx, x):
        return x.view_as(x)

    @staticmethod
    def backward(ctx, dy):
        flush_wgrad_queue()
        return dy


def wgrad_flush_point(x):
    return _FlushPointFn.apply(x) if (_defer_wgrad and x.requires_grad) else x


def _wgrad_into_sink(x, dy, weight, bias, slot, bslot, N, H, W, cin, Ho, Wo, cout, ks, stride):
    M = N * Ho * Wo
    if _defer_wgrad and _async_wgrad and ks == 1 and x.dtype == torch.bfloat16 and M >= 4096:
        _queue_wgrad(x.reshape(M, cin), dy.reshape(M, cout), weight, bias, slot, bslot, M, cin, cout)
        return

    def go():
        _wgrad_launch(x, dy, N, H, W, cin, Ho, Wo, cout, ks, stride, out=slot, dbias=bslot)
        _grad_sink.ready(weight)
        if bslot is not None:
            _grad_sink.ready(bias)

    _off_critical_path((x, dy), go)


def _cache_slot(weight):
    k = id(weight)
    ent = _wcache.get(k)
    if ent is None or ent[0]() is not weight:
        ent = (weakref.ref(weight, lambda _r, k=k: _wcache.pop(k, None)), {})
        _wcache[k] = ent
    return ent[1]


def _round_up(v, m):
    return (v + m - 1) // m * m


def packed_weight(weight: torch.Tensor, bias, dtype: torch.dtype, forward_only: bool = False):
    key = (dtype, "fwd") if forward_only else dtype
    ent = _cache_slot(weight)
    ver = (weight._version, None if bias is None else bias._version, weight.data_ptr(), _pack_epoch)
    if key in ent and ent[key][0] == ver:
        return ent[key][1]
    _require_gpu(weight)
    L = _lib.lib()
    cout, cin = weight.shape[0], weight.shape[1]
    ks = weight.shape[2] if weight.dim() == 4 else 1
    epv = 4 if dtype == torch.float32 else 8
    cin_pad, cout_pad = _round_up(cin, epv), _round_up(cout, epv)
    taps = ks * ks
    w32 = _c(weight.detach().float())
    need_d = cin_pad == cin and not forward_only
    prev = ent[key][1] if key in ent else None
    if prev is not None and prev[0].numel() == cout_pad * taps * cin_pad and prev[0].device == weight.device:
        wf, wd = prev[0], prev[1]
    else:
        wf = torch.empty(cout_pad * taps * cin_pad, dtype=dtype, device=weight.device)
        wd = torch.empty(cin * taps * cout_pad, dtype=dtype, device=weight.device) if need_d else None
        if cout_pad != cout:
            wf.zero_()
    bk = 32 if dtype == torch.float32 else 64
    kbf = bk if (ks == 3 and cin_pad % bk == 0) else 0
    kbd = bk if (ks == 3 and cout_pad % bk == 0) else 0
    _lib.check(
        L.mdm_pack_weight(_p(w32), _p(wf), _p(wd), cout, cin, ks, cin_pad, cout_pad, kbf, kbd,
                          F32 if dtype == torch.float32 else BF16, _stream()),
        "mdm_pack_weight",
    )
    _repacked(wf, wd)
    bp = None
    if bias is not None:
        bp = bias.detach().float()
        if cout_pad != cout:
            bp = torch.cat([bp, bp.new_zeros(cout_pad - cout)])
        bp = _c(bp)
    val = (wf, wd, bp, cin_pad, cout_pad, kbf, kbd)
    ent[key] = (ver, val)
    return val


def packed_s2_dgrad_weight(weight: torch.Tensor):
    ent = _cache_slot(weight)
    ver = (weight._version, weight.data_ptr(), _pack_epoch)
    if "s2dgrad" in ent and ent["s2dgrad"][0] == ver:
        return ent["s2dgrad"][1]
    cout, cin = weight.shape[0], weight.shape[1]
    w = weight.detach()
    if w.dtype != torch.float32 or not w.is_contiguous():
        w = w.float().contiguous()
    old = ent.get("s2dgrad")
    packed = old[1] if old is not None and old[1].shape == (4 * cin, cout // 64, 4, 64) else \
        torch.empty((4 * cin, cout // 64, 4, 64), dtype=torch.bfloat16, device=w.device)
    _lib.check(_lib.lib().mdm_s2dgrad_pack(_p(w), _p(packed), cout, cin, _stream()), "mdm_s2dgrad_pack")
    ent["s2dgrad"] = (ver, packed)
    return packed


_multi_tables = {}


# ... 71 lines not shown
        a[1] += work
        a[2] += e0.elapsed_time(e1) * 1e-3
        a[3] += executed
    if not agg:
        return None
    table = {k: {"launches": v[0], "alg_tflop": round(v[1] / 1e12, 3), "time_ms": round(v[2] * 1e3, 3),
                 "tflops": round(v[1] / v[2] / 1e12, 1)} for k, v in agg.items()}
    for k, v in agg.items():
        if abs(v[3] - v[1]) > 1e-6 * v[1]:
            table[k]["executed_tflops"] = round(v[3] / v[2] / 1e12, 1)
            table[k]["tflops_is"] = "credit for the dense 3x3 layer this sub-pixel kernel replaces (%.2fx the FLOPs it executes)" % (v[1] / v[3])
    dom = max(agg, key=lambda k: agg[k][2])
    n, fl, t = agg[dom][:3]
    ach = fl / t / 1e12
    tot_f, tot_t = sum(v[1] for v in agg.values()), sum(v[2] for v in agg.values())
    return {
        "bound": "mfma", "achieved": round(ach, 1), "peak": peak_tflops, "unit": "TFLOP/s", "frac": round(ach / peak_tflops, 4),
        "traffic": None, "kernel": dom, "dominant_by": "largest total time among the GEMM-class kernels of one step",
        "launches_per_step": n, "avg_launch_ms": round(t / n * 1e3, 4),
        "alg_gflop_per_launch": round(fl / n / 1e9, 2),
        "gemm_weighted": {"alg_tflop": round(tot_f / 1e12, 2), "time_ms": round(tot_t * 1e3, 2),
                          "tflops": round(tot_f / tot_t / 1e12, 1), "frac": round(tot_f / tot_t / 1e12 / peak_tflops, 4)},
        "all_gemm_kernels": table,
        "hbm_kernels": {k: {"launches": v[0], "alg_gb": round(v[1] / 1e9, 3), "time_ms": round(v[2] * 1e3, 3),
                            "gb_per_s": round(v[1] / v[2] / 1e9, 1), "frac_of_peak": round(v[1] / v[2] / 1e9 / peak_gbs, 4)}
                        for k, v in hbm.items()},
    }


_conv_plans = {}


def _conv_plan(M, Cout, K, dt):
    key = (M, Cout, K, dt)
    ent = _conv_plans.get(key)
    if ent is None:
        sp, wsb = ctypes.c_int(1), ctypes.c_size_t(0)
        _lib.check(_lib.lib().mdm_conv_fwd_plan(M, Cout, K, dt, ctypes.byref(sp), ctypes.byref(wsb)), "mdm_conv_fwd_plan")
        ent = _conv_plans[key] = (sp.value, wsb.value)
    return ent


def _repacked(*packs):
    for t in packs:
        if t is not None:
            t._mdm_serial = getattr(t, "_mdm_serial", 0) + 1


def _weight_planes(w: torch.Tensor):
    ent, serial = getattr(w, "_mdm_planes", None), getattr(w, "_mdm_serial", 0)
    if ent is not None and ent[0] == serial:
        return ent[1]
    planes = torch.empty_like(w)
    _lib.check(_lib.lib().mdm_split_weight_planes(_p(w), _p(planes), w.numel(), _stream()), "mdm_split_weight_planes")
    w._mdm_planes = (serial, planes)
    return planes


def _conv_launch(x, w, bias, res, aux, y, ypre, N, H, W, Cin, Ho, Wo, Cout, ks, stride, transposed, act, kblk=0):
    splits, wsb = _conv_plan(N * Ho * Wo, Cout, ks * ks * Cin, _dt(x)) if (stride == 1 and not transposed) else (1, 0)
    ws = _f32_ws(wsb, x.device) if splits > 1 else None
    dt = _dt_mm(x)
    if dt == F32_SPLIT and (ks * ks * Cin) % 8 == 0 and w.numel() % 8 == 0 and _weight_planes_on:
        w, dt = _weight_planes(w), F32_SPLIT_W

    def go():
        _lib.check(
            _lib.lib().mdm_conv_fwd_ws(_p(x), _p(w), _p(bias), _p(res), _p(aux), _p(y), _p(ypre), N, H, W, Cin, Ho, Wo, Cout,
                                       ks, stride, transposed, act, kblk, dt, _p(ws), wsb, _stream()),
            "mdm_conv_fwd",
        )

    if _prof is None:
        return go()
    code = _lib.lib().mdm_conv_fwd_tile(N * Ho * Wo, Cout, _dt(x))
    mode = "1x1" if ks == 1 else ("3x3_T2" if transposed else "3x3")
    name = "conv_gemm_kernel<%s,%dx%d,%s>" % ("f32" if x.dtype == torch.float32 else "bf16", code // 1000, code % 1000, mode)
    flops = 2.0 * N * Ho * Wo * Cout * ks * ks * Cin / (4 if transposed else 1)
    if _prof_shapes:
        name += " M=%d N=%d K=%d" % (N * Ho * Wo, Cout, ks * ks * Cin)
    return _prof_wrap(name, flops, go)


def _wgrad_launch(x, dy, N, H, W, Cin, Ho, Wo, Cout, ks, stride, out=None, dbias=None):
    L = _lib.lib()
    splits = ctypes.c_int(0)
    wsb = ctypes.c_size_t(0)
    M, K = N * Ho * Wo, ks * ks * Cin
    _lib.check(L.mdm_conv_wgrad_plan(M, Cout, K, _dt(x), ctypes.byref(splits), ctypes.byref(wsb)), "mdm_conv_wgrad_plan")
    ws = _f32_ws(wsb.value, x.device)
    dw = torch.empty((Cout, Cin, ks, ks), dtype=torch.float32, device=x.device) if out is None else out

    def go():
        _lib.check(L.mdm_conv_wgrad(_p(x), _p(dy), 0 if dbias is None else 1, _p(ws), N, H, W, Cin, Ho, Wo, Cout, ks, stride,
                                    _dt(x), _stream()),
                   "mdm_conv_wgrad")

    if _prof is None:
        go()
    else:
        te = L.mdm_conv_wgrad_tile(M, Cout, K, _dt(x))
        kn = "conv_wgrad_kernel" if x.dtype == torch.float32 else "conv_wgrad_tr_kernel"
        name = "%s<%s,%dx%d,%s>" % (kn, "f32" if x.dtype == torch.float32 else "bf16", te, te, "1x1" if ks == 1 else "3x3")
        if _prof_shapes:
            name += " M=%d N=%d K=%d" % (M, Cout, K)
        _prof_wrap(name, 2.0 * M * Cout * K, go)
    _lib.check(L.mdm_conv_wgrad_reduce(_p(ws), _p(dw), _p(dbias), _p(dy), M, Cin, Cout, ks, 0 if out is None else 1, _dt(x),
                                       _stream()), "mdm_conv_wgrad_reduce")
    return dw


def _colsum_launch(x2d, M, C, out=None):
    L = _lib.lib()
    nb = ctypes.c_int(0)
    wsb = ctypes.c_size_t(0)
    _lib.check(L.mdm_colsum_plan(M, C, ctypes.byref(nb), ctypes.byref(wsb)), "mdm_colsum_plan")
    ws = _f32_ws(wsb.value, x2d.device)
    acc = 0 if out is None else 1
    if out is None:
        out = torch.empty(C, dtype=torch.float32, device=x2d.device)
    _lib.check(L.mdm_colsum(_p(x2d), _p(out), _p(ws), M, C, acc, _dt(x2d), _stream()), "mdm_colsum")
    return out


def _geom(x, ks, stride):
    if x.dim() == 2:
        return x.shape[0], 1, 1, 1, 1
    N, H, W = x.shape[0], x.shape[1], x.shape[2]
    if ks == 1:
        return N, H, W, H, W
    return N, H, W, (H - 1) // stride + 1, (W - 1) // stride + 1


def _out_shape(x, Ho, Wo, C):
    return (x.shape[0], C) if x.dim() == 2 else (x.shape[0], Ho, Wo, C)


def _conv_forward(x, weight, bias, residual, stride):
    ks = weight.shape[2] if weight.dim() == 4 else 1
    wf, wd, bp, cin_pad, cout_pad, kbf, kbd = packed_weight(weight, bias, x.dtype)
    if x.shape[-1] != cin_pad:
        raise _lib.MdmHipError("conv input has %d channels, packed weight expects %d" % (x.shape[-1], cin_pad))
    N, H, W, Ho, Wo = _geom(x, ks, stride)
    y = torch.empty(_out_shape(x, Ho, Wo, cout_pad), dtype=x.dtype, device=x.device)
    _conv_launch(x, wf, bp, residual, None, y, None, N, H, W, cin_pad, Ho, Wo, cout_pad, ks, stride, 0, 0, kbf)
    return y, ks


class ConvFn(torch.autograd.Function):

    @staticmethod
    def forward(ctx, x, weight, bias, residual, stride, tap=False):
        _require_gpu(x)
        x = _c(x)
        residual = _c(residual)
        y, ks = _conv_forward(x, weight, bias, residual, stride)
        ctx.save_for_backward(x, weight, bias)
        ctx.stride, ctx.ks = stride, ks
        ctx.has_res = residual is not None
        if tap:
            ctx.set_materialize_grads(False)
            return y, x.view_as(x)
        return y

    @staticmethod
    def backward(ctx, dy, dtap=None):
        x, weight, bias = ctx.saved_tensors
        if dy is None:
            raise _lib.MdmHipError("conv(tap=True): the convolution's own output received no gradient")
        return _conv_backward(ctx, x, weight, bias, dy, dtap) + (None, None)


def _conv_backward(ctx, x, weight, bias, dy, dtap=None):
    dy = _c(dy)
    dtap = _c(dtap)
    ks, stride = ctx.ks, ctx.stride
    wf, wd, bp, cin_pad, cout_pad, kbf, kbd = packed_weight(weight, bias, x.dtype)
    cout, cin = weight.shape[0], weight.shape[1]
    N, H, W, Ho, Wo = _geom(x, ks, stride)
    dx = dw = db = None
    if ctx.needs_input_grad[0]:
        if wd is None:
            raise _lib.MdmHipError("input gradient requested for a channel-padded convolution")
        dx = torch.empty_like(x)
        if ks == 3 and stride == 2 and x.dtype == torch.bfloat16 and cout_pad == cout and cout % 64 == 0 and cin % 128 == 0 \
                and H % 2 == 0 and W % 2 == 0:
            wsel = packed_s2_dgrad_weight(weight)
            _prof_wrap("conv_gemm_bl_kernel<sel4> (3x3 stride-2 input gradient) M=%d N=%d K=%d" % (N * Ho * Wo, 4 * cin, 4 * cout),
                       2.0 * N * Ho * Wo * cout * 9 * cin, lambda: _lib.check(
                _lib.lib().mdm_conv_s2_dgrad_res(_p(dy), _p(wsel), _p(dtap), _p(dx), N, Ho, Wo, cout, cin, BF16, _stream()),
                "mdm_conv_s2_dgrad_res"), executed=2.0 * N * Ho * Wo * (4 * cin) * (4 * cout))
            dtap = None
        elif ks == 3 and stride == 2:
            _conv_launch(dy, wd, None, None, None, dx, None, N, Ho, Wo, cout_pad, H, W, cin, 3, 1, 1, 0, kbd)
        else:
            _conv_launch(dy, wd, None, None, None, dx, None, N, Ho, Wo, cout_pad, H, W, cin, ks, 1, 0, 0, kbd)
        if dtap is not None:
            dx = dx + dtap
    elif dtap is not None:
        dx = dtap
    padded = cout_pad != cout or cin_pad != cin
    want_b = bias is not None and ctx.needs_input_grad[2]
    if ctx.needs_input_grad[1]:
        slot = None if padded else _slot(weight)
        bslot = _slot(bias) if (slot is not None and want_b) else None
        if slot is not None:
            _wgrad_into_sink(x, dy, weight, bias, slot, bslot, N, H, W, cin_pad, Ho, Wo, cout_pad, ks, stride)
            if bslot is not None:
                want_b = False
        else:
            dbt = torch.empty(cout_pad, dtype=torch.float32, device=x.device) if want_b else None
            dwp = _wgrad_launch(x, dy, N, H, W, cin_pad, Ho, Wo, cout_pad, ks, stride, dbias=dbt)
            if padded:
                dwp = dwp[:cout, :cin].contiguous()
            dw = dwp.view(weight.shape)
            if want_b:
                db = dbt[:cout]
                want_b = False
    if want_b:
        slot = None if cout_pad != cout else _slot(bias)
        if slot is not None:
            _colsum_launch(dy, N * Ho * Wo, cout_pad, out=slot)
            _grad_sink.ready(bias)
        else:
            db = _colsum_launch(dy, N * Ho * Wo, cout_pad)[:cout]
    dres = dy if (ctx.has_res and ctx.needs_input_grad[3]) else None
    return dx, dw, db, dres


def conv(x, weight, bias=None, residual=None, stride=1):
    return ConvFn.apply(x, weight, bias, residual, stride)


def conv_tap(x, weight, bias=None, stride=1):
    if not (torch.is_grad_enabled() and x.requires_grad):
        return ConvFn.apply(x, weight, bias, None, stride), x
    return ConvFn.apply(x, weight, bias, None, stride, True)


STEM_DGRAD_MAX_CIN = 8


def conv3x3_stem_dgrad(dy, weight, bias=None):
    _require_gpu(dy)
    dy = _c(dy)
    if weight.dim() != 4 or weight.shape[2] != 3 or weight.shape[3] != 3:
        raise _lib.MdmHipError("conv3x3_stem_dgrad: a 3x3 convolution weight is expected")
    cin = weight.shape[1]
    if not 1 <= cin <= STEM_DGRAD_MAX_CIN:
        raise _lib.MdmHipError("input gradient of a channel-padded stem convolution is implemented for at most %d input "
                               "channels (got %d)" % (STEM_DGRAD_MAX_CIN, cin))
    wf, _, _, cin_pad, cout_pad, kbf, _ = packed_weight(weight, bias, dy.dtype)
    if dy.dim() != 4 or dy.shape[-1] != cout_pad or kbf:
        raise _lib.MdmHipError("conv3x3_stem_dgrad: dy %s does not match the packed weight (%d channels)"
                               % (tuple(dy.shape), cout_pad))
    N, H, W = dy.shape[0], dy.shape[1], dy.shape[2]
    dx = torch.empty((N, cin, H, W), dtype=torch.float32, device=dy.device)

    def go():
        _lib.check(_lib.lib().mdm_conv3x3_stem_dgrad(_p(dy), _p(wf), _p(dx), N, H, W, cout_pad, cin, _dt(dy), _stream()),
                   "mdm_conv3x3_stem_dgrad")

    if _prof is None:
        go()
    else:
        name = "stem_dgrad_kernel<%s,%d>" % ("f32" if dy.dtype == torch.float32 else "bf16", cin)
        if _prof_shapes:
            name += " M=%d N=%d K=%d" % (N * H * W, cin, 9 * cout_pad)
        _prof_wrap(name, float(dy.numel() * dy.element_size() + dx.numel() * 4), go, kind="hbm")
    return dx


class StemConvFn(torch.autograd.Function):

    @staticmethod
    def forward(ctx, x, weight, bias, dtype):
        _require_gpu(x)
        x = _c(x.float())
        N, C, H, W = x.shape
        epv = 4 if dtype == torch.float32 else 8
        xh = torch.empty((N, H, W, _round_up(C, epv)), dtype=dtype, device=x.device)
        _lib.check(_lib.lib().mdm_nchw_to_nhwc(_p(x), _p(xh), N, C, H, W, xh.shape[-1], _dt(xh), _stream()), "mdm_nchw_to_nhwc")
        y, _ = _conv_forward(xh, weight, bias, None, 1)
        ctx.save_for_backward(xh, weight, bias)
        return y

    @staticmethod
    def backward(ctx, dy):
        xh, weight, bias = ctx.saved_tensors
        nig = ctx.needs_input_grad
        dy = _c(dy)
        dx = conv3x3_stem_dgrad(dy, weight, bias) if nig[0] else None
        _, dw, db, _ = _conv_backward(_ConvNeeds(3, 1, False, (False, nig[1], nig[2], False)), xh, weight, bias, dy)
        return dx, dw, db, None


def stem_conv(x_nchw, weight, bias=None, dtype=torch.float32):
    if weight.dim() != 4 or weight.shape[2] != 3:
        raise _lib.MdmHipError("stem_conv: a 3x3 convolution weight is expected")
    cin = weight.shape[1]
    if x_nchw.dim() != 4 or x_nchw.shape[1] != cin:
        raise _lib.MdmHipError("stem_conv: input %s vs weight %s" % (tuple(x_nchw.shape), tuple(weight.shape)))
    if cin > STEM_DGRAD_MAX_CIN:
        if cin % (4 if dtype == torch.float32 else 8) == 0:
            return conv(to_nhwc(x_nchw, dtype), weight, bias)
# ... 2 lines not shown
    return StemConvFn.apply(x_nchw, weight, bias, dtype)


def packed_upconv_weights(weight: torch.Tensor, bias):
    ent = _cache_slot(weight)
    ver = (weight._version, None if bias is None else bias._version, weight.data_ptr(), _pack_epoch)
    if "upconv" in ent and ent["upconv"][0] == ver:
        return ent["upconv"][1]
    cout, cin = weight.shape[0], weight.shape[1]
    prev = ent["upconv"][1] if "upconv" in ent else None
    if prev is not None and prev[0].device == weight.device:
        w_ph, w_t = prev[0], prev[1]
    else:
        w_ph = torch.empty(4 * cout * 4 * cin, dtype=torch.bfloat16, device=weight.device)
        w_t = torch.empty(cin * 16 * cout, dtype=torch.bfloat16, device=weight.device)
    _lib.check(_lib.lib().mdm_upconv_pack(_p(_c(weight.detach().float())), _p(w_ph), _p(w_t), cout, cin, _stream()), "mdm_upconv_pack")
    bias4 = _c(bias.detach().float().repeat(4)) if bias is not None else None
    val = (w_ph, w_t, bias4)
    ent["upconv"] = (ver, val)
    return val


def upsample_conv_supported(x, weight):
    return x.is_cuda and x.dtype == torch.bfloat16 and x.dim() == 4 and weight.dim() == 4 and weight.shape[2] == 3 and \
        weight.shape[0] % 256 == 0 and weight.shape[1] % 256 == 0 and x.shape[-1] == weight.shape[1] and \
        (x.shape[1] & (x.shape[1] - 1)) == 0 and (x.shape[2] & (x.shape[2] - 1)) == 0


class UpsampleConvFn(torch.autograd.Function):

    @staticmethod
    def forward(ctx, x, weight, bias):
        _require_gpu(x)
        x = _c(x)
        N, H, W, cin = x.shape
        cout = weight.shape[0]
        w_ph, _, bias4 = packed_upconv_weights(weight, bias)
        y = torch.empty((N, 2 * H, 2 * W, cout), dtype=x.dtype, device=x.device)
        _prof_wrap("conv_gemm_bl_kernel<sel4> (upsample2x + 3x3) M=%d N=%d K=%d" % (N * H * W, 4 * cout, 4 * cin),
                   2.0 * N * 4 * H * W * cout * 9 * cin, lambda: _lib.check(
            _lib.lib().mdm_conv_up_fwd(_p(x), _p(w_ph), _p(bias4), _p(y), N, H, W, cin, cout, BF16, _stream()), "mdm_conv_up_fwd"),
                   executed=2.0 * N * H * W * (4 * cout) * (4 * cin))
        ctx.save_for_backward(x, weight, bias)
        return y

    @staticmethod
    def backward(ctx, dy):
        x, weight, bias = ctx.saved_tensors
        dy = _c(dy)
        N, H, W, cin = x.shape
        cout = weight.shape[0]
        L = _lib.lib()
        _, w_t, _ = packed_upconv_weights(weight, bias)
        dyb = torch.empty((N, H, W, 4 * cout), dtype=dy.dtype, device=dy.device)
        _lib.check(L.mdm_space_to_depth2x(_p(dy), _p(dyb), N, H, W, cout, BF16, _stream()), "mdm_space_to_depth2x")
        dx = dw = db = None
        if ctx.needs_input_grad[0]:
            dx = torch.empty_like(x)
            _prof_wrap("conv_gemm_bl_kernel<sel4> (upsample2x + 3x3 input gradient) M=%d N=%d K=%d" % (N * H * W, cin, 16 * cout),
                       2.0 * N * 4 * H * W * cout * 9 * cin, lambda: _lib.check(
                L.mdm_conv_up_dgrad(_p(dyb), _p(w_t), _p(dx), N, H, W, cout, cin, BF16, _stream()), "mdm_conv_up_dgrad"),
                           executed=2.0 * N * H * W * cin * (16 * cout))
        if ctx.needs_input_grad[1]:
            want_b = bias is not None and ctx.needs_input_grad[2]
            slot = _slot(weight)
            bslot = _slot(bias) if (slot is not None and want_b) else None
            sunk = slot is not None and (bslot is not None or not want_b)
            M, K = N * H * W, 9 * cin
            splits, wsb = ctypes.c_int(0), ctypes.c_size_t(0)
            _lib.check(L.mdm_conv_wgrad_plan(M, 4 * cout, K, BF16, ctypes.byref(splits), ctypes.byref(wsb)), "mdm_conv_wgrad_plan")

            def go():
                ws = _f32_ws(wsb.value, x.device)
                dwb = torch.empty((4 * cout, cin, 3, 3), dtype=torch.float32, device=x.device)
                db4 = torch.empty(4 * cout, dtype=torch.float32, device=x.device) if want_b else None
                _prof_wrap("conv_wgrad_bl_kernel<1, 1> (upsample2x + 3x3, 16 of 36 blocks) M=%d N=%d K=%d" % (M, 4 * cout, K),
                           2.0 * 4 * M * cout * K, lambda: _lib.check(
                    L.mdm_conv_wgrad_blocked(_p(x), _p(dyb), 1 if want_b else 0, _p(ws), N, H, W, cin, cout, BF16, _stream()),
                    "mdm_conv_wgrad_blocked"), executed=2.0 * 4 * M * cout * K * 16.0 / 36.0)
                _lib.check(L.mdm_conv_wgrad_reduce(_p(ws), _p(dwb), _p(db4), _p(dyb), M, cin, 4 * cout, 3, 0, BF16, _stream()),
                           "mdm_conv_wgrad_reduce")
                dwo = slot if sunk else torch.empty(weight.shape, dtype=torch.float32, device=x.device)
                dbo = (bslot if sunk else torch.empty(cout, dtype=torch.float32, device=x.device)) if want_b else None
                _lib.check(L.mdm_upconv_wfold(_p(dwb), _p(dwo), _p(db4), _p(dbo), cout, cin, 1 if sunk else 0, _stream()), "mdm_upconv_wfold")
                if sunk:
                    _grad_sink.ready(weight)
                    if want_b:
                        _grad_sink.ready(bias)
                return dwo, dbo

            if sunk:
                _off_critical_path((x, dyb), go)
            else:
                dw, db = go()
        return dx, dw, db


def upsample_conv(x, weight, bias=None):
    if upsample_conv_supported(x, weight):
        return UpsampleConvFn.apply(x, weight, bias)
    return ConvFn.apply(upsample2x(x), weight, bias, None, 1)


def linear(x, weight, bias=None, residual=None):
    shp = x.shape
    y = ConvFn.apply(x.reshape(-1, shp[-1]), weight, bias, None if residual is None else residual.reshape(-1, weight.shape[0]), 1)
    return y.reshape(*shp[:-1], weight.shape[0])


class FFNFn(torch.autograd.Function):

    @staticmethod
    def forward(ctx, x, w1, b1, w2, b2, residual, keep):
        _require_gpu(x)
        x, residual = _c(x), _c(residual)
        wf1, _, bp1, c_in, c_hid, _, _ = packed_weight(w1, b1, x.dtype)
        wf2, _, bp2, _, c_out, _, _ = packed_weight(w2, b2, x.dtype)
        N, H, W, _, _ = _geom(x, 1, 1)
        byte_code = x.dtype == torch.bfloat16 and _lib.lib().mdm_dev_ffn_aux_bytes() == 1
        pre = torch.empty(_out_shape(x, H, W, c_hid), dtype=torch.uint8 if byte_code else x.dtype, device=x.device) if keep else None
        a = torch.empty(_out_shape(x, H, W, c_hid), dtype=x.dtype, device=x.device)
        _conv_launch(x, wf1, bp1, None, None, a, pre, N, H, W, c_in, H, W, c_hid, 1, 1, 0, 1)
        y = torch.empty(_out_shape(x, H, W, c_out), dtype=x.dtype, device=x.device)
        _conv_launch(a, wf2, bp2, residual, None, y, None, N, H, W, c_hid, H, W, c_out, 1, 1, 0, 0)
        ctx.save_for_backward(x, w1, b1, w2, b2, pre, a)
        ctx.has_res = residual is not None
        return y

    @staticmethod
    def backward(ctx, dy):
        x, w1, b1, w2, b2, pre, a = ctx.saved_tensors
        dy = _c(dy)
        _, wd1, _, c_in, c_hid, _, _ = packed_weight(w1, b1, x.dtype)
        _, wd2, _, _, c_out, _, _ = packed_weight(w2, b2, x.dtype)
        N, H, W, _, _ = _geom(x, 1, 1)
        M = N * H * W
        dpre = torch.empty_like(a)
        _conv_launch(dy, wd2, None, None, pre, dpre, None, N, H, W, c_out, H, W, c_hid, 1, 1, 0, 2)
        def wb_grads(xin, g, w, b, cin_, cout_):
            sw, sb = _slot(w), _slot(b)
            if sw is not None and sb is not None:
                _wgrad_into_sink(xin, g, w, b, sw, sb, N, H, W, cin_, H, W, cout_, 1, 1)
                return None, None
            dbt = torch.empty(cout_, dtype=torch.float32, device=xin.device)
            return _wgrad_launch(xin, g, N, H, W, cin_, H, W, cout_, 1, 1, dbias=dbt).view(w.shape), dbt

        dw1 = db1 = dw2 = db2 = None
        if ctx.needs_input_grad[3] or ctx.needs_input_grad[4]:
            dw2, db2 = wb_grads(a, dy, w2, b2, c_hid, c_out)
        dx = None
        if ctx.needs_input_grad[0]:
            dx = torch.empty_like(x)
            _conv_launch(dpre, wd1, None, None, None, dx, None, N, H, W, c_hid, H, W, c_in, 1, 1, 0, 0)
        if ctx.needs_input_grad[1] or ctx.needs_input_grad[2]:
            dw1, db1 = wb_grads(x, dpre, w1, b1, c_in, c_hid)
        dres = dy if (ctx.has_res and ctx.needs_input_grad[5]) else None
        return dx, dw1, db1, dw2, db2, dres, None


def ffn(x, w1, b1, w2, b2, residual):
    return FFNFn.apply(x, w1, b1, w2, b2, residual, torch.is_grad_enabled())


_adapter_epoch = 0


def adapter_epoch() -> int:
# ... 382 lines not shown
            bp = None
        elif bp is not None and bp.shape == bias.shape and bp.device == bias.device:
            bp.copy_(bias.detach())
        else:
            bp = bias.detach().float().contiguous().clone()
    ent["mx8_3x3"] = (ver, (wq, bp))
    return ent["mx8_3x3"][1]


def _gn_ws(N, HW, C, G, device):
    wsb = ctypes.c_size_t(0)
    _lib.check(_lib.lib().mdm_gn_plan(N, HW, C, G, ctypes.byref(wsb)), "mdm_gn_plan")
    return _f32_ws(wsb.value, device)


def _gn_forward(x, gamma, beta, film, groups, eps, act):
    N, C = x.shape[0], x.shape[-1]
    HW = x.numel() // (N * C)
    g32, b32 = _c(gamma.detach().float()), _c(beta.detach().float())
    y = torch.empty_like(x)
    stats = torch.empty((N, groups, 2), dtype=torch.float32, device=x.device)
    coef = torch.empty((N, C, 2), dtype=torch.float32, device=x.device)
    ws = _gn_ws(N, HW, C, groups, x.device)
    _prof_wrap("group_norm fwd (HW=%d)" % HW, 2.0 * x.numel() * x.element_size(), lambda: _lib.check(
        _lib.lib().mdm_gn_fwd(_p(x), _p(g32), _p(b32), _p(film), _p(y), _p(stats), _p(coef), _p(ws), N, HW, C,
                              groups, float(eps), act, _dt(x), _stream()),
        "mdm_gn_fwd",
    ), kind="hbm")
    return y, stats, coef


class GroupNormFn(torch.autograd.Function):

    @staticmethod
    def forward(ctx, x, gamma, beta, film, groups, eps, act, passthrough):
        _require_gpu(x)
        x, film = _c(x), _c(film)
        y, stats, coef = _gn_forward(x, gamma, beta, film, groups, eps, act)
        ctx.save_for_backward(x, gamma, beta, film, stats, coef)
        ctx.groups, ctx.act = groups, act
        ctx.passthrough = passthrough
        ctx.set_materialize_grads(False)
        if passthrough == 2:
            return y, x.view_as(x), x.view_as(x)
        if passthrough:
            return y, x.view_as(x)
        return y

    @staticmethod
    def backward(ctx, dy, dres=None, dres2=None):
        x, gamma, beta, film, stats, coef = ctx.saved_tensors
        if dy is None:
            dy = torch.zeros_like(x)
        dx, dgamma, dbeta, dfilm = _gn_backward(dy, x, gamma, beta, film, stats, coef, dres, dres2, ctx.groups, ctx.act,
                                                ctx.needs_input_grad[1] or ctx.needs_input_grad[2])
        return dx, dgamma, dbeta, dfilm, None, None, None, None


def _gn_backward(dy, x, gamma, beta, film, stats, coef, dres, dres2, groups, act, need_params=True):
    dy = _c(dy)
    dres = _c(dres) if dres is not None else None
    dres2 = _c(dres2) if dres2 is not None else None
    if dres is None and dres2 is not None:
        dres, dres2 = dres2, None
    N, C = x.shape[0], x.shape[-1]
    HW = x.numel() // (N * C)
    g32, b32 = _c(gamma.detach().float()), _c(beta.detach().float())
    dx = torch.empty_like(x)
    sg, sb = _slot(gamma), _slot(beta)
    sunk = sg is not None and sb is not None
    deferred = sunk and _defer_wgrad
    rows = need_params and not sunk and N >= 3
    if deferred:
        dgamma, dbeta = _gn_rows(N, C, x.device)
    elif rows:
        dgamma = torch.empty((N, C), dtype=torch.float32, device=x.device)
        dbeta = torch.empty((N, C), dtype=torch.float32, device=x.device)
    else:
        dgamma = sg if sunk else torch.empty(C, dtype=torch.float32, device=x.device)
        dbeta = sb if sunk else torch.empty(C, dtype=torch.float32, device=x.device)
    dfilm = torch.empty_like(film) if film is not None else None
    ws = _gn_ws(N, HW, C, groups, x.device)
    mode = 2 if (deferred or rows) else (1 if sunk else 0)
    npass = 3.0 + (dres is not None) + (dres2 is not None)
    _prof_wrap("group_norm bwd (HW=%d)" % HW, npass * x.numel() * x.element_size(), lambda: _lib.check(
        _lib.lib().mdm_gn_bwd(_p(dy), _p(x), _p(g32), _p(b32), _p(film), _p(stats), _p(coef), _p(dres), _p(dres2), _p(dx), _p(dgamma),
                              _p(dbeta), _p(dfilm), _p(ws), N, HW, C, groups, act, mode, _dt(x), _stream()),
        "mdm_gn_bwd",
    ), kind="hbm")
    if deferred:
        _gn_pending.append((dgamma, dbeta, sg, sb, N, C, gamma, beta))
        _sink_defer(gamma)
        _sink_defer(beta)
        return dx, None, None, dfilm
    if sunk:
        _grad_sink.ready(gamma)
        _grad_sink.ready(beta)
        return dx, None, None, dfilm
    if not need_params:
        return dx, None, None, dfilm
    if rows:
        pg, pb = dgamma, dbeta
        dgamma, dbeta = _prof_wrap("group_norm param rows sum (wgrad of gamma / beta, N=%d)" % N, 2.0 * 4 * (N + 1) * C,
                                   lambda: (pg.sum(0), pb.sum(0)), kind="hbm")
    return dx, dgamma, dbeta, dfilm


def group_norm(x, gamma, beta, groups, eps=1e-5, film=None, silu=False, passthrough=False):
    return GroupNormFn.apply(x, gamma, beta, film, groups, eps, 1 if silu else 0, int(passthrough))


_act_recompute = False


def enable_activation_recompute(flag: bool):
    global _act_recompute
    _act_recompute = bool(flag)


def activation_recompute_enabled() -> bool:
    return _act_recompute


def gn_reapply(x, coef, silu=True, p=0.0, seed=0, offset=0):
    _require_gpu(x)
    x = _c(x)
    N, C = x.shape[0], x.shape[-1]
    if tuple(coef.shape) != (N, C, 2) or coef.dtype != torch.float32 or coef.device != x.device:
        raise _lib.MdmHipError("gn_reapply: coef must be fp32 [N=%d, C=%d, 2] on %s, got %s %s on %s" % (
            N, C, x.device, coef.dtype, tuple(coef.shape), coef.device))
    coef = _c(coef)
    HW = x.numel() // (N * C)
    y = torch.empty_like(x)
    nbytes = 2.0 * x.numel() * x.element_size()
    _prof_wrap("group_norm reapply (HW=%d)" % HW, nbytes, lambda: _lib.check(
        _lib.lib().mdm_gn_reapply(_p(x), _p(coef), _p(y), N, HW, C, 1 if silu else 0, float(p), int(seed), int(offset), _dt(x),
                                  _stream()), "mdm_gn_reapply"), kind="hbm")
    return y


class _ConvNeeds:

    __slots__ = ("ks", "stride", "has_res", "needs_input_grad")

    def __init__(self, ks, stride, has_res, needs):
        self.ks, self.stride, self.has_res, self.needs_input_grad = ks, stride, has_res, needs


class GnConvFn(torch.autograd.Function):

    @staticmethod
    def forward(ctx, x, gamma, beta, film, groups, eps, act, passthrough, p, weight, bias, residual):
        _require_gpu(x)
        x, film, residual = _c(x), _c(film), _c(residual)
        h, stats, coef = _gn_forward(x, gamma, beta, film, groups, eps, act)
        seed = off = 0
        if p > 0.0:
            h, seed, off = _dropout_forward(h, p)
        y, ks = _conv_forward(h, weight, bias, residual, 1)
        del h
        ctx.save_for_backward(x, gamma, beta, film, stats, coef, weight, bias)
        ctx.groups, ctx.act, ctx.ks = groups, act, ks
        ctx.has_res = residual is not None
        ctx.drop = (float(p), seed, off)
        ctx.set_materialize_grads(False)
        if passthrough == 2:
            return y, x.view_as(x), x.view_as(x)
        if passthrough:
            return y, x.view_as(x)
        return y

    @staticmethod
    def backward(ctx, dy, dres=None, dres2=None):
        x, gamma, beta, film, stats, coef, weight, bias = ctx.saved_tensors
        if dy is None:
            raise _lib.MdmHipError("gn_conv: the convolution's output received no gradient")
        nig = ctx.needs_input_grad
        need_dh = nig[0] or nig[1] or nig[2] or nig[3]
        p, seed, off = ctx.drop
        if nig[9]:
            h = gn_reapply(x, coef, bool(ctx.act), p, seed, off)
        else:
            h = x
        dh, dw, db, dres_conv = _conv_backward(_ConvNeeds(ctx.ks, 1, ctx.has_res, (need_dh, nig[9], nig[10], nig[11])),
                                               h, weight, bias, dy)
        del h
        dx = dgamma = dbeta = dfilm = None
        if need_dh:
            if p > 0.0:
                dhd = torch.empty_like(dh)
                _lib.check(_lib.lib().mdm_dropout(_p(dh), _p(dhd), dh.numel(), p, seed, off, _dt(dh), _stream()), "mdm_dropout")
                dh = dhd
            dx, dgamma, dbeta, dfilm = _gn_backward(dh, x, gamma, beta, film, stats, coef, dres, dres2, ctx.groups, ctx.act,
                                                    nig[1] or nig[2])
        return dx, dgamma, dbeta, dfilm, None, None, None, None, None, dw, db, dres_conv


def gn_conv(x, gamma, beta, groups, weight, bias=None, eps=1e-5, film=None, silu=True, passthrough=False, p=0.0,
            residual=None):
    if weight.dim() != 4 or weight.shape[2] != 3:
        raise _lib.MdmHipError("gn_conv: a 3x3 convolution weight is expected")
    p = float(p)
    if not 0.0 <= p < 1.0:
        raise _lib.MdmHipError("gn_conv: dropout probability %r outside [0, 1)" % p)
    if p > 0.0 and x.numel() % 8 != 0:
        raise _lib.MdmHipError("dropout: the element count must be a multiple of 8")
    return GnConvFn.apply(x, gamma, beta, film, groups, eps, 1 if silu else 0, int(passthrough), p, weight, bias, residual)


class LayerNormFn(torch.autograd.Function):
    @staticmethod
    def forward(ctx, x, gamma, beta, eps):
        _require_gpu(x)
        x = _c(x)
        D = x.shape[-1]
        R = x.numel() // D
        g32, b32 = _c(gamma.detach().float()), _c(beta.detach().float())
        y = torch.empty_like(x)
        stats = torch.empty((R, 2), dtype=torch.float32, device=x.device)
        _lib.check(_lib.lib().mdm_ln_fwd(_p(x), _p(g32), _p(b32), _p(y), _p(stats), R, D, float(eps), _dt(x), _stream()), "mdm_ln_fwd")
        ctx.save_for_backward(x, gamma, beta, stats)
        return y

    @staticmethod
    def backward(ctx, dy):
        x, gamma, beta, stats = ctx.saved_tensors
        dy = _c(dy)
        D = x.shape[-1]
        R = x.numel() // D
        g32 = _c(gamma.detach().float())
        dx = torch.empty_like(x)
        sg, sb = _slot(gamma), _slot(beta)
        sunk = sg is not None and sb is not None
        dgamma = sg if sunk else torch.empty(D, dtype=torch.float32, device=x.device)
        dbeta = sb if sunk else torch.empty(D, dtype=torch.float32, device=x.device)
        ws = torch.empty(((R + 63) // 64) * D * 2, dtype=torch.float32, device=x.device)
        _lib.check(_lib.lib().mdm_ln_bwd(_p(dy), _p(x), _p(g32), _p(stats), _p(dx), _p(dgamma), _p(dbeta), _p(ws), R, D,
                                         1 if sunk else 0, _dt(x), _stream()), "mdm_ln_bwd")
        if sunk:
            _grad_sink.ready(gamma)
            _grad_sink.ready(beta)
            return dx, None, None, None
        return dx, dgamma, dbeta, None


def layer_norm(x, gamma, beta, eps=1e-5):
    return LayerNormFn.apply(x, gamma, beta, eps)


def _ptr_array(ts):
    return (ctypes.c_void_p * len(ts))(*[_p(t) for t in ts])


class TextKVFn(torch.autograd.Function):

    @staticmethod
    def forward(ctx, cond, eps, *params):
        _require_gpu(cond)
        cond = _c(cond)
        B, S, D = cond.shape
        R, L = B * S, len(params) // 4
        lnw, lnb, ws, bs = params[0::4], params[1::4], params[2::4], params[3::4]
        lib = _lib.lib()
        g32 = [_c(t.detach().float()) for t in lnw]
        b32 = [_c(t.detach().float()) for t in lnb]
        cn = [torch.empty_like(cond) for _ in range(L)]
        stats = torch.empty((R, 2), dtype=torch.float32, device=cond.device)
        _lib.check(lib.mdm_ln_multi_fwd(_p(cond), _ptr_array(g32), _ptr_array(b32), _ptr_array(cn), L, _p(stats), R, D, float(eps),
                                        _dt(cond), _stream()), "mdm_ln_multi_fwd")
        groups = {}
        for l, w in enumerate(ws):
            groups.setdefault(w.shape[0], []).append(l)
        ys = [None] * L
        for cout, idx in groups.items():
            packs = [packed_weight(ws[l], bs[l], cond.dtype) for l in idx]
            for l in idx:
                ys[l] = torch.empty((B, S, cout), dtype=cond.dtype, device=cond.device)
            _prof_wrap("linear grouped x%d M=%d N=%d K=%d" % (len(idx), R, cout, D), 2.0 * len(idx) * R * cout * D, lambda: _lib.check(
                lib.mdm_linear_grouped(_ptr_array([cn[l] for l in idx]), _ptr_array([pk[0] for pk in packs]),
                                       _ptr_array([pk[2] for pk in packs]), _ptr_array([ys[l] for l in idx]), len(idx), R, D, cout,
                                       _dt(cond), _stream()), "mdm_linear_grouped"))
        ctx.save_for_backward(cond, stats, *cn, *params)
        ctx.L, ctx.groups = L, groups
        return tuple(ys)

    @staticmethod
    def backward(ctx, *dys):
        saved = ctx.saved_tensors
        L, groups = ctx.L, ctx.groups
        cond, stats, cn, params = saved[0], saved[1], saved[2:2 + L], saved[2 + L:]
        lnw, lnb, ws, bs = params[0::4], params[1::4], params[2::4], params[3::4]
        B, S, D = cond.shape
        R = B * S
        lib = _lib.lib()
        dys = [_c(d) if d is not None else torch.zeros((B, S, ws[l].shape[0]), dtype=cond.dtype, device=cond.device)
               for l, d in enumerate(dys)]
        dcn = [torch.empty_like(cond) for _ in range(L)]
        grads = [None] * (4 * L)
        def dgrad(cout, idx):
            packs = [packed_weight(ws[l], bs[l], cond.dtype) for l in idx]
            _prof_wrap("linear grouped x%d M=%d N=%d K=%d" % (len(idx), R, D, cout), 2.0 * len(idx) * R * cout * D, lambda: _lib.check(
                lib.mdm_linear_grouped(_ptr_array([dys[l] for l in idx]), _ptr_array([pk[1] for pk in packs]), None,
                                       _ptr_array([dcn[l] for l in idx]), len(idx), R, cout, D, _dt(cond), _stream()),
                "mdm_linear_grouped"))

        nig = ctx.needs_input_grad
        for cout, idx in groups.items():
            if not any(nig[2 + 4 * l + 2] or nig[2 + 4 * l + 3] for l in idx):
                continue
            slots = [(_slot(ws[l]), _slot(bs[l])) for l in idx]
            sunk = all(a is not None and b is not None for a, b in slots)
            if sunk:
                dws, dbs = [a for a, _ in slots], [b for _, b in slots]
            else:
                dws = [torch.zeros(ws[l].shape, dtype=torch.float32, device=cond.device) for l in idx]
                dbs = [torch.zeros(bs[l].shape, dtype=torch.float32, device=cond.device) for l in idx]
            xs2, dy2 = [cn[l].reshape(R, D) for l in idx], [dys[l].reshape(R, cout) for l in idx]

            def go(xs2=xs2, dy2=dy2, dws=dws, dbs=dbs, idx=idx, sunk=sunk, cout=cout):
                _prof_wrap("conv_wgrad grouped x%d M=%d N=%d K=%d" % (len(idx), R, cout, D), 2.0 * len(idx) * R * cout * D,
                           lambda: wgrad_grouped(xs2, dy2, dws, dbs))
                if sunk:
                    for l in idx:
                        _grad_sink.ready(ws[l])
                        _grad_sink.ready(bs[l])

            if sunk:
                _off_critical_path(xs2 + dy2, go)
            else:
                go()
                for k, l in enumerate(idx):
                    grads[4 * l + 2], grads[4 * l + 3] = dws[k], dbs[k]
        for cout, idx in groups.items():
            dgrad(cout, idx)
        g32 = [_c(t.detach().float()) for t in lnw]
        nslots = [(_slot(lnw[l]), _slot(lnb[l])) for l in range(L)]
        nsunk = all(a is not None and b is not None for a, b in nslots)
        if nsunk:
            dgs, dbs_ = [a for a, _ in nslots], [b for _, b in nslots]
        else:
            dgs = [torch.empty(D, dtype=torch.float32, device=cond.device) for _ in range(L)]
            dbs_ = [torch.empty(D, dtype=torch.float32, device=cond.device) for _ in range(L)]
        dcond = torch.empty_like(cond)
        _lib.check(lib.mdm_ln_multi_bwd(_ptr_array(dcn), _p(cond), _ptr_array(g32), _p(stats), _p(dcond), _ptr_array(dgs),
                                        _ptr_array(dbs_), L, R, D, 1 if nsunk else 0, _dt(cond), _stream()), "mdm_ln_multi_bwd")
        if nsunk:
            for l in range(L):
                _grad_sink.ready(lnw[l])
                _grad_sink.ready(lnb[l])
        else:
            for l in range(L):
                grads[4 * l], grads[4 * l + 1] = dgs[l], dbs_[l]
        return (dcond, None) + tuple(grads)


class SharedInputLinearsFn(torch.autograd.Function):

    @staticmethod
    def forward(ctx, x, *params):
        _require_gpu(x)
        x = _c(x)
        R, D = x.shape
        ws, bs = params[0::2], params[1::2]
        L = len(ws)
        lib = _lib.lib()
        groups = {}
        for l, w in enumerate(ws):
            groups.setdefault(w.shape[0], []).append(l)
        ys = [None] * L
        for cout, idx in groups.items():
            packs = [packed_weight(ws[l], bs[l], x.dtype) for l in idx]
            for l in idx:
                ys[l] = torch.empty((R, cout), dtype=x.dtype, device=x.device)
            _lib.check(lib.mdm_linear_grouped(_ptr_array([x] * len(idx)), _ptr_array([pk[0] for pk in packs]),
                                              _ptr_array([pk[2] for pk in packs]), _ptr_array([ys[l] for l in idx]), len(idx), R, D,
                                              cout, _dt(x), _stream()), "mdm_linear_grouped")
        ctx.save_for_backward(x, *params)
        ctx.groups = groups
        return tuple(ys)

    @staticmethod
    def backward(ctx, *dys):
        x, params = ctx.saved_tensors[0], ctx.saved_tensors[1:]
        ws, bs = params[0::2], params[1::2]
        L, groups = len(ws), ctx.groups
        R, D = x.shape
        lib = _lib.lib()
        dys = [_c(d) if d is not None else torch.zeros((R, ws[l].shape[0]), dtype=x.dtype, device=x.device) for l, d in enumerate(dys)]
        dxs = [torch.empty_like(x) for _ in range(L)]
        grads = [None] * (2 * L)
        def dgrad(cout, idx):
            packs = [packed_weight(ws[l], bs[l], x.dtype) for l in idx]
            _lib.check(lib.mdm_linear_grouped(_ptr_array([dys[l] for l in idx]), _ptr_array([pk[1] for pk in packs]), None,
                                              _ptr_array([dxs[l] for l in idx]), len(idx), R, cout, D, _dt(x), _stream()),
                       "mdm_linear_grouped")

        nig = ctx.needs_input_grad
        for cout, idx in groups.items():
            if not any(nig[1 + 2 * l] or nig[2 + 2 * l] for l in idx):
                continue
            slots = [(_slot(ws[l]), _slot(bs[l])) for l in idx]
            sunk = all(a is not None and b is not None for a, b in slots)
            if sunk:
                dws, dbs = [a for a, _ in slots], [b for _, b in slots]
            else:
                dws = [torch.zeros(ws[l].shape, dtype=torch.float32, device=x.device) for l in idx]
                dbs = [torch.zeros(bs[l].shape, dtype=torch.float32, device=x.device) for l in idx]
            xs2, dy2 = [x] * len(idx), [dys[l] for l in idx]

            def go(xs2=xs2, dy2=dy2, dws=dws, dbs=dbs, idx=idx, sunk=sunk, cout=cout):
                _prof_wrap("conv_wgrad grouped x%d M=%d N=%d K=%d" % (len(idx), R, cout, D), 2.0 * len(idx) * R * cout * D,
                           lambda: wgrad_grouped(xs2, dy2, dws, dbs))
                if sunk:
                    for l in idx:
                        _grad_sink.ready(ws[l])
                        _grad_sink.ready(bs[l])

            if sunk:
                _off_critical_path([x] + dy2, go)
            else:
                go()
                for k, l in enumerate(idx):
                    grads[2 * l], grads[2 * l + 1] = dws[k], dbs[k]
        for cout, idx in groups.items():
            dgrad(cout, idx)
        dx = dxs[0] if L == 1 else torch.stack(dxs).sum(0)
        return (dx,) + tuple(grads)


def shared_input_linears_supported(x, layers):
    return x.is_cuda and x.dtype == torch.bfloat16 and x.dim() == 2 and x.shape[-1] % 64 == 0 and 0 < len(layers) and \
        all(w.shape[0] % 64 == 0 and b is not None for w, b in layers) and \
        max(sum(1 for w2, _ in layers if w2.shape[0] == w.shape[0]) for w, _ in layers) <= 32


def shared_input_linears(x, layers):
    return SharedInputLinearsFn.apply(x, *[t for pair in layers for t in pair])


def text_kv_supported(cond, layers):
    return cond.is_cuda and cond.dtype == torch.bfloat16 and cond.shape[-1] % 64 == 0 and 0 < len(layers) <= 32 and \
        all(w.shape[0] % 64 == 0 for _, _, w, _ in layers)


def text_kv(cond, layers, eps=1e-5):
    flat = [t for quad in layers for t in quad]
    return TextKVFn.apply(cond, eps, *flat)


class AttentionFn(torch.autograd.Function):

    @staticmethod
    def forward(ctx, qkv, kvc, mask, heads, keep):
        _require_gpu(qkv)
        qkv, kvc = _c(qkv), _c(kvc)
        B = qkv.shape[0]
        C = qkv.shape[-1] // 3
        L = qkv.numel() // (B * 3 * C)
        S = kvc.shape[1] if kvc is not None else 0
        d = C // heads
        m32 = _c(mask.float()) if mask is not None else None
        out = torch.empty(qkv.shape[:-1] + (C,), dtype=qkv.dtype, device=qkv.device)
        lse_s = torch.empty((B, heads, L), dtype=torch.float32, device=qkv.device) if keep else None
        lse_c = torch.empty((B, heads, L), dtype=torch.float32, device=qkv.device) if (keep and kvc is not None) else None
        oc = torch.empty_like(out) if kvc is not None else None
        _prof_wrap("attn_fwd_kernel<d=%d> L=%d" % (d, L), 4.0 * B * heads * L * (L + S) * d, lambda: _lib.check(
            _lib.lib().mdm_attn_fwd(_p(qkv), _p(kvc), _p(m32), _p(out), _p(oc), _p(lse_s), _p(lse_c), B, L, S, heads, d, _dt_mm(qkv), _stream()),
            "mdm_attn_fwd",
        ), kind="attn")
        ctx.save_for_backward(qkv, kvc, m32, out, oc, lse_s, lse_c)
        ctx.heads = heads
        return out

    @staticmethod
    def backward(ctx, dout):
        qkv, kvc, m32, out, oc, lse_s, lse_c = ctx.saved_tensors
        dout = _c(dout)
        B = qkv.shape[0]
        C = qkv.shape[-1] // 3
        L = qkv.numel() // (B * 3 * C)
        S = kvc.shape[1] if kvc is not None else 0
        heads = ctx.heads
        d = C // heads
        dqkv = torch.empty_like(qkv)
        dkvc = torch.empty_like(kvc) if kvc is not None else None
        delta_s = torch.empty_like(lse_s)
        delta_c = torch.empty_like(lse_c) if kvc is not None else None
        _prof_wrap("attn_bwd (delta + dq + dkv kernels)<d=%d> L=%d" % (d, L), 8.0 * B * heads * L * (L + S) * d, lambda: _lib.check(
            _lib.lib().mdm_attn_bwd(_p(qkv), _p(kvc), _p(m32), _p(out), _p(oc), _p(dout), _p(lse_s), _p(lse_c), _p(delta_s),
                                    _p(delta_c), _p(dqkv), _p(dkvc), B, L, S, heads, d, _dt(qkv), _stream()),
            "mdm_attn_bwd",
        ), kind="attn")
        return dqkv, dkvc, None, None, None


# ... 808 lines not shown
        ctx.save_for_backward(pred, x_t, images, eps, g)
        ctx.cfg = (float(inv_scale), ptype, ttype)
        return loss

    @staticmethod
    def backward(ctx, gloss):
        pred, x_t, images, eps, g = ctx.saved_tensors
        inv_scale, ptype, ttype = ctx.cfg
        B = pred.shape[0]
        chw = pred.numel() // B
        gl = _vec(gloss, B)
        dpred = torch.empty_like(pred)
        _lib.check(_lib.lib().mdm_diffusion_loss_bwd(_p(x_t), _p(pred), _p(images), _p(eps), _p(g), _p(gl), inv_scale, _p(dpred),
                                                     B, chw, ptype, ttype, _stream()), "mdm_diffusion_loss_bwd")
        return dpred, None, None, None, None, None, None, None


def diffusion_loss(pred, x_t, images, eps, g, prediction_type, target_type, inv_scale=1.0):
    if pred.dtype != torch.float32:
        raise _lib.MdmHipError("diffusion_loss: the model output at the boundary is fp32 (got %s)" % pred.dtype)
    return DiffusionLossFn.apply(pred, x_t, images, eps, g, float(inv_scale), _ptype(prediction_type), _ptype(target_type))


def avgpool(x, r):
    x = _img(x)
    N, C, H, W = x.shape
    y = torch.empty((N, C, H // r, W // r), dtype=torch.float32, device=x.device)
    _lib.check(_lib.lib().mdm_avgpool(_p(x), _p(y), N, C, H, W, int(r), _stream()), "mdm_avgpool")
    return y


class SampleStdFn(torch.autograd.Function):

    @staticmethod
    def forward(ctx, x):
        x = _img(x)
        N = x.shape[0]
        chw = x.numel() // N
        y = torch.empty_like(x)
        stats = torch.empty((N, 2), dtype=torch.float32, device=x.device)
        ws = torch.empty(N * 64 * 2, dtype=torch.float32, device=x.device)
        _lib.check(_lib.lib().mdm_sample_std_fwd(_p(x), _p(y), _p(stats), _p(ws), N, chw, _stream()), "mdm_sample_std_fwd")
        ctx.save_for_backward(x, stats)
        return y

    @staticmethod
    def backward(ctx, dy):
        x, stats = ctx.saved_tensors
        dy = _c(dy.float())
        N = x.shape[0]
        chw = x.numel() // N
        dx = torch.empty_like(x)
        ws = torch.empty(N * 64 * 2, dtype=torch.float32, device=x.device)
        _lib.check(_lib.lib().mdm_sample_std_bwd(_p(dy), _p(x), _p(stats), _p(dx), _p(ws), N, chw, _stream()), "mdm_sample_std_bwd")
        return dx


def sample_std_normalize(x):
    return SampleStdFn.apply(x)


def input_stage(u8_nhwc):
    _require_gpu(u8_nhwc)
    if u8_nhwc.dtype != torch.uint8 or u8_nhwc.dim() != 4 or u8_nhwc.shape[-1] != 3:
        raise _lib.MdmHipError("input_stage: expected a uint8 [B, H, W, 3] tensor")
    u = _c(u8_nhwc)
    B, H, W, _ = u.shape
    out = torch.empty((B, 3, H, W), dtype=torch.float32, device=u.device)
    _lib.check(_lib.lib().mdm_input_stage(_p(u), _p(out), B, H, W, _stream()), "mdm_input_stage")
    return out


def sumsq(flat_f32, out=None, step_counter=None):
    _require_gpu(flat_f32)
    out = torch.empty(1, dtype=torch.float32, device=flat_f32.device) if out is None else out
    ws = torch.empty(1024, dtype=torch.float32, device=flat_f32.device)
    _lib.check(_lib.lib().mdm_sumsq(_p(flat_f32), _p(out), _p(ws), flat_f32.numel(), _p(step_counter), _stream()), "mdm_sumsq")
    return out


def adamw_ema_step(p, g, m, v, ema, gnorm_sq, lr, beta1, beta2, eps, weight_decay, step, clip, ema_decay, zero_grad=True,
                   step_dev=None):
    _require_gpu(p)
    nbytes = 4.0 * p.numel() * ((4 if ema is None else 5) + (3 if ema is None else 4) + (1 if zero_grad else 0))
    _prof_wrap("adamw_ema_step", nbytes, lambda: _lib.check(
        _lib.lib().mdm_adamw_ema_step(_p(p), _p(g), _p(m), _p(v), _p(ema), _p(gnorm_sq), p.numel(), float(lr), float(beta1),
                                      float(beta2), float(eps), float(weight_decay), int(step), _p(step_dev), float(clip), float(ema_decay),
                                      1 if zero_grad else 0, _stream()),
        "mdm_adamw_ema_step",
    ), kind="hbm")
    invalidate_packed_weights()


_dropout_rng = [None, 0]


def seed_dropout(seed: int, rank: int = None):
    if rank is None:
        rank = torch.distributed.get_rank() if (torch.distributed.is_available() and torch.distributed.is_initialized()) else 0
    _dropout_rng[0] = (int(seed) + 0x9E3779B97F4A7C15 * int(rank)) & 0xFFFFFFFFFFFFFFFF
    _dropout_rng[1] = 0


def get_dropout_rng_state():
    if _dropout_rng[0] is None:
        seed_dropout(torch.initial_seed())
    return (_dropout_rng[0], _dropout_rng[1])


def set_dropout_rng_state(state):
    _dropout_rng[0], _dropout_rng[1] = int(state[0]) & 0xFFFFFFFFFFFFFFFF, int(state[1])


def _dropout_forward(x, p):
    if _dropout_rng[0] is None:
        seed_dropout(torch.initial_seed())
    seed, off = _dropout_rng
    _dropout_rng[1] = off + (x.numel() + 3) // 4
    y = torch.empty_like(x)
    _lib.check(_lib.lib().mdm_dropout(_p(x), _p(y), x.numel(), float(p), seed, off, _dt(x), _stream()), "mdm_dropout")
    return y, seed, off


class DropoutFn(torch.autograd.Function):
    @staticmethod
    def forward(ctx, x, p):
        _require_gpu(x)
        y, seed, off = _dropout_forward(_c(x), p)
        ctx.p, ctx.seed, ctx.off = float(p), seed, off
        return y

    @staticmethod
    def backward(ctx, dy):
        dy = _c(dy)
        dx = torch.empty_like(dy)
        _lib.check(_lib.lib().mdm_dropout(_p(dy), _p(dx), dy.numel(), ctx.p, ctx.seed, ctx.off, _dt(dy), _stream()), "mdm_dropout")
        return dx, None


def dropout(x, p: float, training: bool = True):
    if not training or p <= 0.0:
        return x
    if p >= 1.0:
        return x * 0.0
    if x.numel() % 8 != 0:
        raise _lib.MdmHipError("dropout: the element count must be a multiple of 8")
    return DropoutFn.apply(x, p)
```

### ml-mdm_amd/mdm_hip/trainer.py

```python
import collections
import math
import os

import torch

from . import ops
from .distributed import DataParallel, GradReducer


class FusedState:

    def __init__(self, net, reducer=None, bucket_mb=256.0, wire_dtype="auto", use_ema=True, async_wgrad=True):
        self.net = net
        self.params = [p for p in net.parameters() if p.requires_grad]
        late = net.late_gradient_parameters() if hasattr(net, "late_gradient_parameters") else None
        self.reducer = reducer if reducer is not None else GradReducer(self.params, bucket_mb=bucket_mb, wire_dtype=wire_dtype,
                                                                       late_params=late)
        self.reducer.broadcast_parameters(0)
        flat = torch.empty_like(self.reducer.flat)
        self.slices = {}
        off = 0
        with torch.no_grad():
            for p in self.reducer.order:
                n = p.numel()
                flat[off:off + n].copy_(p.reshape(-1))
                p.data = flat[off:off + n].view_as(p)
                self.slices[id(p)] = (off, n)
                off += n
        self.flat_p = flat
        self.m = torch.zeros_like(flat)
        self.v = torch.zeros_like(flat)
        self.flat_ema = flat.clone() if use_ema else None
        self.gnorm_sq = torch.zeros(1, dtype=torch.float32, device=flat.device)
        self.step_dev = torch.zeros(1, dtype=torch.int32, device=flat.device)
        self.reducer.rebind()
        self.async_wgrad = async_wgrad
        self._host_vals = {}
        self.activate()

    def activate(self):
        ops.set_grad_sink(self.reducer)
        ops.enable_async_wgrad(self.async_wgrad)
        ops.enable_deferred_wgrad(self.async_wgrad, max_group=32 if self.reducer.world == 1 else 13)
        ops.invalidate_packed_weights()

    def view(self, arena, p):
        off, n = self.slices[id(p)]
        return arena[off:off + n].view_as(p)

    def finish_backward(self):
        ops.flush_wgrad_queue()
        self.reducer.mark("bw1")
        ops.join_side_stream()
        self.reducer.finish()

    def post_scalar(self, name, value):
        ent = self._host_vals.get(name)
        if ent is None:
            ent = (torch.empty(1, dtype=torch.float32).pin_memory(), torch.cuda.Event())
            self._host_vals[name] = ent
        ent[0].copy_(value.detach().reshape(1), non_blocking=True)
        ent[1].record()

    def read_scalar(self, name):
        buf, ev = self._host_vals[name]
        ev.synchronize()
        return float(buf[0])

    def post_skip_flag(self):
        ring = self.__dict__.setdefault("_skip_ring", [])
        k = self.__dict__.get("_skip_next", 0)
        if len(ring) <= k:
            ring.append((torch.empty(1, dtype=torch.float32).pin_memory(), torch.cuda.Event()))
        buf, ev = ring[k]
        self._skip_next = (k + 1) % 4
        buf.copy_(self.gnorm_sq.detach().reshape(1), non_blocking=True)
        ev.record()
        return buf, ev

    def optimizer_step(self, lr, betas, eps, weight_decay, clip_norm, ema_decay, dtype, loss=None):
        if loss is not None and self.reducer.world == 1:
            self.reducer.flat[:1].add_(loss.detach().float().reshape(1) * 0.0)
        ops.sumsq(self.reducer.flat, out=self.gnorm_sq, step_counter=self.step_dev)
        ops.adamw_ema_step(self.flat_p, self.reducer.flat, self.m, self.v, self.flat_ema, self.gnorm_sq, lr, betas[0], betas[1],
                           eps, weight_decay, 0, clip_norm, ema_decay, zero_grad=True, step_dev=self.step_dev)
        ops.repack_all(dtype)


def _vision_model(model):
    core = getattr(model.model, "module", model.model)
    return core.vision_model


def _adopt(model, optimizer, ema_model):
    st = getattr(optimizer, "_mdm_fused", None)
    if st is not None:
        if st is not False and st.ema_id != (id(ema_model) if ema_model is not None else None):
            raise RuntimeError("train_batch was first called %s and now %s: pass the same ema_model on every call "
                               "(the fused step adopted it together with the optimizer)"
                               % ("without an ema_model" if st.ema_id is None else "with another ema_model",
                                  "without one" if ema_model is None else "with one"))
        return st if st is not False else None

    def no(reason):
        optimizer._mdm_fused = False
        optimizer._mdm_fused_reason = reason
        return None

    from .unet import UNet

    wrapped = model.model
    net = _vision_model(model)
    if isinstance(wrapped, torch.nn.parallel.DistributedDataParallel):
        return no("torch DistributedDataParallel owns the gradient buckets (use mdm_hip.distributed.DataParallel)")
    if not isinstance(net, UNet):
        return no("vision model is not an mdm_hip UNet")
    params = [p for p in net.parameters() if p.requires_grad]
    if not params:
        return no("vision model has no trainable parameters")
    if not all(p.is_cuda and p.dtype == torch.float32 for p in params):
        return no("parameters are not fp32 tensors on the GPU")
    if type(optimizer) not in (torch.optim.AdamW, torch.optim.Adam) or len(optimizer.param_groups) != 1:
        return no("optimizer is not a single-group torch Adam / AdamW")
    grp = optimizer.param_groups[0]
    if grp.get("amsgrad") or grp.get("maximize") or (type(optimizer) is torch.optim.Adam and grp.get("weight_decay", 0) != 0
                                                      and not grp.get("decoupled_weight_decay", False)):
        return no("optimizer options without a fused counterpart (amsgrad / maximize / L2 weight decay)")
    if [id(p) for p in grp["params"]] != [id(p) for p in params]:
        return no("optimizer does not hold exactly the vision model's parameters")
    ema_net = None
    if ema_model is not None:
        ema_net = ema_model.module
        if getattr(ema_model, "device", None) is not None or set(net.state_dict()) != {n for n, _ in net.named_parameters()} or \
                [(n, tuple(p.shape)) for n, p in ema_net.named_parameters()] != [(n, tuple(p.shape)) for n, p in net.named_parameters()]:
            return no("ModelEma on another device / of another shape / with persistent buffers")
    reducer = wrapped.reducer if isinstance(wrapped, DataParallel) else \
        GradReducer(params, group=None, world_override=1)
    if [id(p) for p in reducer.params] != [id(p) for p in params]:
        return no("the DataParallel wrapper's reducer does not hold exactly the vision model's parameters")
    had_state = {id(p): dict(optimizer.state.get(p, {})) for p in params}
    st = FusedState(net, reducer=reducer, use_ema=ema_net is not None, async_wgrad=os.environ.get("MDM_HIP_SERIAL_WGRAD", "0") != "1")
    with torch.no_grad():
        steps = 0
        for p in params:
            old = had_state[id(p)]
            mv, vv = st.view(st.m, p), st.view(st.v, p)
            if "exp_avg" in old:
                mv.copy_(old["exp_avg"])
                vv.copy_(old["exp_avg_sq"])
                steps = max(steps, int(old["step"]))
            optimizer.state[p] = {"step": None, "exp_avg": mv, "exp_avg_sq": vv}
        st.step_dev.fill_(steps)
        step_host = torch.tensor(float(steps))
        for p in params:
            optimizer.state[p]["step"] = step_host
        optimizer.register_state_dict_pre_hook(lambda opt, st=st, t=step_host: (_settle(st, keep=0), t.fill_(float(int(st.step_dev)))) and None)

        def _reinstall(opt, st=st, params=params, t=step_host):
            with torch.no_grad():
                steps_ = 0
                for p_ in params:
                    ent = opt.state.get(p_)
                    if not ent or "exp_avg" not in ent:
                        continue
                    mv_, vv_ = st.view(st.m, p_), st.view(st.v, p_)
                    if ent["exp_avg"].data_ptr() != mv_.data_ptr():
                        mv_.copy_(ent["exp_avg"])
                        vv_.copy_(ent["exp_avg_sq"])
# ... 287 lines not shown
```

Measured before the change: 11.42 steps/s.

## Overwrite gradient slots on first write instead of zeroing the flat gradient buffer

Tracks which parameters have already received a gradient this step. The first producer of each gradient writes it directly instead of accumulating into it, so the optimizer no longer zeroes the whole flat gradient buffer every step. Parameters that have additive producers, or that were not written this step, are zeroed lazily through a new batched range-fill kernel. This removes one full write pass over the gradient buffer in the AdamW kernel, at the cost of host-side bookkeeping per wgrad launch and a risk of stale gradients if the tracking misses a case.

After: 11.50 steps/s (median of 6 runs). About the same (+0.7%).

```diff
diff --git a/include/mdm_hip_ext.h b/include/mdm_hip_ext.h
--- a/include/mdm_hip_ext.h
+++ b/include/mdm_hip_ext.h
@@ -3,6 +3,10 @@
 #ifdef __cplusplus
 extern "C" {
 #endif
+
+int mdm_conv_wgrad_grouped_ow(const void* const* x, const void* const* dy, float* const* dw, float* const* dbias,
+                              int groups, int overwrite_mask, int M, int Cin, int Cout, int dtype, void* stream);
+int mdm_fill_zero_ranges(float* base, const void* table, int n, int total_blocks, void* stream);
 
 int mdm_attn_cross_bias(const void* qkv, const void* kvc, const float* mask, const float* bias, int bias_ld,
                         const void* base, int base_ld, void* out, int B, int L, int S, int H, int d, int dtype,
diff --git a/ml-mdm_amd/csrc/gemm_conv.hip b/ml-mdm_amd/csrc/gemm_conv.hip
--- a/ml-mdm_amd/csrc/gemm_conv.hip
+++ b/ml-mdm_amd/csrc/gemm_conv.hip
@@ -609,6 +609,7 @@
   int groups;
   int bias_share;
   int skip_cout;
+  unsigned overwrite;
 };
 
 constexpr int WG_MAXG = 32;
@@ -1318,7 +1319,10 @@
         v += __shfl_xor(v, 32, 64);
         const int n = n0 + wm * TM + (wn * BR + r) * 16 + l16;
         if (quad == 0 && n < p.Cout) {
-          if (p.groups > 0) gr.bout[grp][n] += v;
+          if (p.groups > 0) {
+            if ((p.overwrite >> grp) & 1u) gr.bout[grp][n] = v;
+            else gr.bout[grp][n] += v;
+          }
           else p.bslab[((size_t)split * bias_share + kt_rel) * p.Cout + n] = v;
         }
       }
@@ -1341,9 +1345,10 @@
   if (bias_blk && p.groups == 0 && split == 0 && kt_rel == 0 && n0 == 0 && tid == 0)
     reinterpret_cast<int*>(p.bslab - WG_BHDR)[0] = bias_share;
   const bool direct = p.groups > 0;
+  const bool add = direct && !((p.overwrite >> grp) & 1u);
   float* __restrict__ S = direct ? gr.out[grp] : p.slab + (size_t)split * p.Cout * p.K;
   const bool vec_ok = (p.K & 3) == 0;
-  if (!direct) {
+  if (!add) {
 #pragma unroll
     for (int i = 0; i < MT; ++i) {
       const int n = n0 + wm * TM + i * 16 + l16;
@@ -2632,14 +2637,14 @@
   return 0;
 }
 
-extern "C" int mdm_conv_wgrad_grouped(const void* const* x, const void* const* dy, float* const* dw,
-                                      float* const* dbias, int groups, int M, int Cin, int Cout, int dtype,
-                                      void* stream) {
+static int wgrad_grouped_launch(const void* const* x, const void* const* dy, float* const* dw, float* const* dbias,
+                                int groups, unsigned overwrite, int M, int Cin, int Cout, int dtype, void* stream) {
   MDM_CHECK_ARG(x && dy && dw && groups >= 1 && groups <= WG_MAXG);
   MDM_CHECK_ARG(dtype == DT_BF16 && Cin % 8 == 0 && Cout % 8 == 0 && M > 0);
   WgradArgs a = {};
   a.N = M; a.H = 1; a.W = 1; a.Cin = Cin; a.Ho = 1; a.Wo = 1; a.Cout = Cout; a.stride = 1;
   a.M = M; a.K = Cin; a.splits = 1; a.groups = groups;
+  a.overwrite = groups < 32 ? overwrite & ((1u << groups) - 1u) : overwrite;
   a.mtiles_per_split = (M + 63) / 64;
   MDM_CHECK_ARG(wgrad_bl_ok(a, 1));
   WgradGroup gr = {};
@@ -2662,6 +2667,18 @@
   }
   MDM_NOTE_KERNEL("conv_wgrad_bl_kernel<%d, %d>", MODE_1x1, te == 256 ? 1 : 0);
   MDM_LAUNCH_STATUS();
+}
+
+extern "C" int mdm_conv_wgrad_grouped(const void* const* x, const void* const* dy, float* const* dw,
+                                      float* const* dbias, int groups, int M, int Cin, int Cout, int dtype,
+                                      void* stream) {
+  return wgrad_grouped_launch(x, dy, dw, dbias, groups, 0u, M, Cin, Cout, dtype, stream);
+}
+
+extern "C" int mdm_conv_wgrad_grouped_ow(const void* const* x, const void* const* dy, float* const* dw,
+                                         float* const* dbias, int groups, int overwrite_mask, int M, int Cin,
+                                         int Cout, int dtype, void* stream) {
+  return wgrad_grouped_launch(x, dy, dw, dbias, groups, (unsigned)overwrite_mask, M, Cin, Cout, dtype, stream);
 }
 
 extern "C" int mdm_conv_wgrad_reduce(const float* ws, float* dw_oihw, float* dbias, const void* dy, int M, int Cin,
diff --git a/ml-mdm_amd/csrc/norm.hip b/ml-mdm_amd/csrc/norm.hip
--- a/ml-mdm_amd/csrc/norm.hip
+++ b/ml-mdm_amd/csrc/norm.hip
@@ -1112,7 +1112,8 @@
 struct GnParamDesc {
   const float* pg; const float* pb;
   float* dgamma; float* dbeta;
-  int N, C, first_block, pad_;
+  int N, C, first_block;
+  int overwrite;
 };
 
 __global__ __launch_bounds__(256) void gn_param_reduce_multi_kernel(const GnParamDesc* __restrict__ table, int n) {
@@ -1142,8 +1143,10 @@
   red[0][q][cl] = a; red[1][q][cl] = b;
   __syncthreads();
   if (q == 0 && c < d.C) {
-    d.dgamma[c] += (red[0][0][cl] + red[0][1][cl]) + (red[0][2][cl] + red[0][3][cl]);
-    d.dbeta[c] += (red[1][0][cl] + red[1][1][cl]) + (red[1][2][cl] + red[1][3][cl]);
+    const float sg = (red[0][0][cl] + red[0][1][cl]) + (red[0][2][cl] + red[0][3][cl]);
+    const float sb = (red[1][0][cl] + red[1][1][cl]) + (red[1][2][cl] + red[1][3][cl]);
+    if (d.overwrite & 1) { d.dgamma[c] = sg; d.dbeta[c] = sb; }
+    else { d.dgamma[c] += sg; d.dbeta[c] += sb; }
   }
 }
 
diff --git a/ml-mdm_amd/csrc/optim.hip b/ml-mdm_amd/csrc/optim.hip
--- a/ml-mdm_amd/csrc/optim.hip
+++ b/ml-mdm_amd/csrc/optim.hip
@@ -52,7 +52,7 @@
   const float denom = sqrtf(v) / sqrtf(a.bc2) + a.eps;
   p -= (a.lr / a.bc1) * (m / denom);
   if (has_ema) e = e * a.ema_decay + p * (1.f - a.ema_decay);
-  if (a.zero_grad) g = 0.f;
+  if (a.zero_grad == 1) g = 0.f;
 }
 
 __global__ __launch_bounds__(256) void adamw_ema_kernel(AdamArgs a) {
@@ -94,7 +94,7 @@
     }
     p4[i] = p; m4[i] = m; v4[i] = v;
     if (has_ema) e4[i] = e;
-    if (a.zero_grad) g4[i] = g;
+    if (a.zero_grad == 1) g4[i] = g;
   }
   if (blockIdx.x == 0) {
     for (size_t i = n4 * 4 + threadIdx.x; i < a.n; i += 256) {
@@ -105,9 +105,47 @@
   }
 }
 
+struct FillRange {
+  unsigned long long off;
+  unsigned count;
+  unsigned first_block;
+};
+constexpr unsigned FILL_BLOCK = 16384;
+
+__global__ __launch_bounds__(256) void fill_zero_ranges_kernel(float* __restrict__ base, const FillRange* __restrict__ table,
+                                                               int n) {
+  int lo = 0, hi = n - 1;
+  while (lo < hi) {
+    const int mid = (lo + hi + 1) >> 1;
+    if (table[mid].first_block <= blockIdx.x) lo = mid; else hi = mid - 1;
+  }
+  const FillRange r = table[lo];
+  const size_t end = (size_t)r.off + r.count;
+  const size_t first = (size_t)r.off + (size_t)(blockIdx.x - r.first_block) * FILL_BLOCK;
+  if (first >= end) return;
+  const size_t last = first + FILL_BLOCK < end ? first + FILL_BLOCK : end;
+  size_t a0 = (first + 3) & ~(size_t)3;
+  if (a0 > last) a0 = last;
+  size_t a1 = last & ~(size_t)3;
+  if (a1 < a0) a1 = a0;
+  for (size_t i = first + threadIdx.x; i < a0; i += 256) base[i] = 0.f;
+  f32x4* b4 = reinterpret_cast<f32x4*>(base);
+  for (size_t i = a0 / 4 + threadIdx.x; i < a1 / 4; i += 256) b4[i] = f32x4{0.f, 0.f, 0.f, 0.f};
+  for (size_t i = a1 + threadIdx.x; i < last; i += 256) base[i] = 0.f;
+}
+
 }
 
 using namespace mdm;
+
+extern "C" int mdm_fill_zero_ranges(float* base, const void* table, int n, int total_blocks, void* stream) {
+  MDM_CHECK_ARG(base && table && n > 0 && total_blocks > 0);
+  MDM_CHECK_ARG(((size_t)base & 15) == 0 && ((size_t)table & 7) == 0);
+  static_assert(sizeof(FillRange) == 16, "record layout is part of the ABI");
+  hipLaunchKernelGGL(fill_zero_ranges_kernel, dim3(total_blocks), dim3(256), 0, reinterpret_cast<hipStream_t>(stream), base,
+                     (const FillRange*)table, n);
+  MDM_LAUNCH_STATUS();
+}
 
 extern "C" int mdm_sumsq(const float* g, float* out, float* ws, size_t n, int* step_counter, void* stream) {
   MDM_CHECK_ARG(g && out && ws);
diff --git a/ml-mdm_amd/mdm_hip/distributed.py b/ml-mdm_amd/mdm_hip/distributed.py
--- a/ml-mdm_amd/mdm_hip/distributed.py
+++ b/ml-mdm_amd/mdm_hip/distributed.py
@@ -44,11 +44,30 @@
         dist.barrier()
 
 
+FILL_BLOCK = 16384
+
+
+def fill_range_table(ranges, device):
+    import numpy as np
+    rng = []
+    for o, n in ranges:
+        while n > 0:
+            c = min(n, 1 << 30)
+            rng.append((o, c))
+            o, n = o + c, n - c
+    rec = np.zeros(len(rng), dtype=[("off", "<u8"), ("count", "<u4"), ("first", "<u4")])
+    blocks = 0
+    for k, (o, n) in enumerate(rng):
+        rec[k] = (o, n, blocks)
+        blocks += (n + FILL_BLOCK - 1) // FILL_BLOCK
+    return torch.from_numpy(rec.view(np.uint8).copy()).to(device), blocks
+
+
 class GradReducer:
 
     def __init__(self, params, bucket_mb: float = 256.0, wire_dtype="auto", group=None, tail_mb: float = 8.0,
                  world_override: int = None, force_collectives: bool = False, head_mb: float = 64.0,
-                 record_timeline: bool = False, late_params=None):
+                 record_timeline: bool = False, late_params=None, force_accumulate: bool = False):
         self.params = [p for p in params if p.requires_grad]
         self.group = group
         self.nranks = dist.get_world_size(group) if dist.is_initialized() else 1
@@ -101,6 +120,19 @@
         if off > b_start:
             self.buckets.append((b_start, off))
         self._slots = {p.data_ptr(): (p, p.grad) for p in self.params}
+        self._pos = {}
+        self._span = []
+        o = 0
+        for i, p in enumerate(order):
+            self._pos[id(p)] = i
+            self._span.append((o, p.numel()))
+            o += p.numel()
+        self._written = set()
+        self._stale = set()
+        self._adders = set()
+        self._fill_tables = {}
+        self.force_accumulate = bool(force_accumulate)
+        self.fill_stats = {"launches": 0, "cache_hits": 0, "full_zero": 0}
         self._grad_ptrs = [(p, p.grad.data_ptr()) for p in self.params]
         self._need = [0] * len(self.buckets)
         for p in order:
@@ -129,6 +161,102 @@
 
     def rebind(self):
         self._slots = {p.data_ptr(): (p, p.grad) for p in self.params}
+
+    def _idx(self, p):
+        ent = self._slots.get(p.data_ptr())
+        return None if ent is None else self._pos[id(ent[0])]
+
+    def claim(self, *params):
+        idx = [self._idx(p) for p in params if p is not None]
+        if self.force_accumulate or any(i is None for i in idx):
+            self.adding(*params)
+            return False
+        w = self._written
+        if not any(i in w for i in idx):
+            w.update(idx)
+            self._stale.difference_update(idx)
+            return True
+        for i in idx:
+            if i not in w:
+                self._zero_if_stale(i)
+                w.add(i)
+        return False
+
+    def adding(self, *params):
+        for p in params:
+            i = None if p is None else self._idx(p)
+            if i is None:
+                continue
+            if not self.force_accumulate:
+                self._adders.add(i)
+            if i not in self._written:
+                self._zero_if_stale(i)
+
+    def is_written(self, p):
+        return self._idx(p) in self._written
+
+    def is_adder(self, p):
+        return self._idx(p) in self._adders
+
+    def _zero_if_stale(self, i):
+        if i in self._stale:
+            o, n = self._span[i]
+            self.flat[o:o + n].zero_()
+            self._stale.discard(i)
+
+    def _ranges(self, idx):
+        out = []
+        for i in idx:
+            o, n = self._span[i]
+            if n == 0:
+                continue
+            if out and out[-1][0] + out[-1][1] == o:
+                out[-1][1] += n
+            else:
+                out.append([o, n])
+        return [(o, n) for o, n in out]
+
+    def _fill(self, idx):
+        key = tuple(sorted(idx))
+        if not key:
+            return
+        ent = self._fill_tables.get(key)
+        if ent is None:
+            rng = self._ranges(key)
+            table, blocks = fill_range_table(rng, self.flat.device) if (self.flat.is_cuda and rng) else (None, 0)
+            if len(self._fill_tables) > 16:
+                self._fill_tables.clear()
+            ent = self._fill_tables[key] = (table, rng, blocks)
+        else:
+            self.fill_stats["cache_hits"] += 1
+        table, rng, blocks = ent
+        if not rng:
+            return
+        self.fill_stats["launches"] += 1
+        if table is not None:
+            from . import ops
+            ops.fill_zero_ranges(self.flat, table, table.numel() // 16, blocks)
+        else:
+            for o, n in rng:
+                self.flat[o:o + n].zero_()
+
+    def settle(self):
+        if self._stale:
+            gone = self._stale - self._written
+            self._stale.clear()
+            self._fill(gone)
+
+    def zero_unwritten(self):
+        own = self._written | self._stale
+        self._fill([i for i in range(len(self._span)) if i not in own])
+
+    def step_done(self):
+        self._stale = self._written
+        self._written = set()
+        self.zero_unwritten()
+
+    def release(self):
+        self.settle()
 
     def _hook(self, p):
         if id(p) in self._deferred:
@@ -288,6 +416,9 @@
 
     def zero_grad(self):
         self.flat.zero_()
+        self._written = set()
+        self._stale = set()
+        self.fill_stats["full_zero"] += 1
 
     def broadcast_parameters(self, src: int = 0):
         if self.nranks == 1:
diff --git a/ml-mdm_amd/mdm_hip/ops.py b/ml-mdm_amd/mdm_hip/ops.py
--- a/ml-mdm_amd/mdm_hip/ops.py
+++ b/ml-mdm_amd/mdm_hip/ops.py
@@ -106,6 +106,9 @@
     global _grad_sink
     if _grad_sink is not None and sink is not _grad_sink:
         flush_wgrad_queue()
+        rel = getattr(_grad_sink, "release", None)
+        if rel is not None:
+            rel()
     _grad_sink = sink
 
 
@@ -113,6 +116,22 @@
     if _grad_sink is None or param is None:
         return None
     return _grad_sink.slot(param)
+
+
+def _claim(*params):
+    f = getattr(_grad_sink, "claim", None)
+    return 0 if (f is not None and f(*params)) else 1
+
+
+def _adding(*params):
+    f = getattr(_grad_sink, "adding", None)
+    if f is not None:
+        f(*params)
+
+
+def fill_zero_ranges(base, table, n, blocks):
+    _require_gpu(base)
+    _lib.check(_lib.lib().mdm_fill_zero_ranges(_p(base), _p(table), int(n), int(blocks), _stream()), "mdm_fill_zero_ranges")
 
 
 def _sink_defer(param):
@@ -184,7 +203,15 @@
     _WG_MAX = max(1, min(32, int(max_group)))
 
 
-def wgrad_grouped(xs, dys, dws, dbs=None):
+def _ow_mask(flags):
+    m = 0
+    for g, f in enumerate(flags):
+        if f:
+            m |= 1 << g
+    return m - (1 << 32) if m >= (1 << 31) else m
+
+
+def wgrad_grouped(xs, dys, dws, dbs=None, overwrite=None):
     G = len(xs)
     M, cin = xs[0].shape
     cout = dys[0].shape[1]
@@ -192,6 +219,13 @@
         _require_gpu(t)
     xs, dys = [_c(t) for t in xs], [_c(t) for t in dys]
     arr = lambda vals: (ctypes.c_void_p * G)(*vals)
+    if overwrite is not None and any(overwrite):
+        _lib.check(_lib.lib().mdm_conv_wgrad_grouped_ow(arr([_p(t) for t in xs]), arr([_p(t) for t in dys]),
+                                                        arr([_p(t) for t in dws]),
+                                                        arr([_p(t) for t in dbs]) if dbs is not None else None, G,
+                                                        _ow_mask(overwrite), M, cin, cout, _dt(xs[0]), _stream()),
+                   "mdm_conv_wgrad_grouped_ow")
+        return
     _lib.check(_lib.lib().mdm_conv_wgrad_grouped(arr([_p(t) for t in xs]), arr([_p(t) for t in dys]), arr([_p(t) for t in dws]),
                                                  arr([_p(t) for t in dbs]) if dbs is not None else None, G, M, cin, cout,
                                                  _dt(xs[0]), _stream()), "mdm_conv_wgrad_grouped")
@@ -217,15 +251,16 @@
     tile = ctypes.c_int(0)
     _lib.check(L.mdm_conv_wgrad_group_plan(M, cout, cin, BF16, len(q), ctypes.byref(tile)), "mdm_conv_wgrad_group_plan")
     tensors = [t for e in q for t in (e[0], e[1])]
-    if tile.value and all((e[5] is not None) == (q[0][5] is not None) for e in q):
+    if tile.value and all((e[5] is not None) == (q[0][5] is not None) for e in q) and len({e[4].data_ptr() for e in q}) == len(q):
         G = len(q)
         arr = lambda vals: (ctypes.c_void_p * G)(*vals)
         xs, dys, dws = arr([_p(e[0]) for e in q]), arr([_p(e[1]) for e in q]), arr([_p(e[4]) for e in q])
         dbs = arr([_p(e[5]) for e in q]) if q[0][5] is not None else None
 
         def go():
+            mask = _ow_mask([_claim(e[2], e[3] if e[5] is not None else None) == 0 for e in q])
             _prof_wrap("conv_wgrad grouped x%d M=%d N=%d K=%d" % (G, M, cout, cin), 2.0 * G * M * cout * cin, lambda: _lib.check(
-                L.mdm_conv_wgrad_grouped(xs, dys, dws, dbs, G, M, cin, cout, BF16, _stream()), "mdm_conv_wgrad_grouped"))
+                L.mdm_conv_wgrad_grouped_ow(xs, dys, dws, dbs, G, mask, M, cin, cout, BF16, _stream()), "mdm_conv_wgrad_grouped_ow"))
             for e in q:
                 _grad_sink.ready(e[2])
                 if e[5] is not None:
@@ -233,7 +268,8 @@
     else:
         def go():
             for x, dy, w, b, slot, bslot in q:
-                _wgrad_launch(x, dy, M, 1, 1, cin, 1, 1, cout, 1, 1, out=slot, dbias=bslot)
+                _wgrad_launch(x, dy, M, 1, 1, cin, 1, 1, cout, 1, 1, out=slot, dbias=bslot,
+                              accumulate=_claim(w, b if bslot is not None else None))
                 _grad_sink.ready(w)
                 if bslot is not None:
                     _grad_sink.ready(b)
@@ -267,15 +303,16 @@
     if not _gn_pending:
         return
     dev = _gn_pending[0][0].device
-    key = tuple((e[0].data_ptr(), e[1].data_ptr(), e[2].data_ptr(), e[3].data_ptr(), e[4], e[5]) for e in _gn_pending)
+    key = tuple((e[0].data_ptr(), e[1].data_ptr(), e[2].data_ptr(), e[3].data_ptr(), e[4], e[5], 1 - _claim(e[6], e[7]))
+                for e in _gn_pending)
     ent = _gn_tables.get(key)
     if ent is None:
         import numpy as np
         rec = np.zeros(len(key), dtype=[("pg", "<u8"), ("pb", "<u8"), ("dg", "<u8"), ("db", "<u8"), ("N", "<i4"),
-                                         ("C", "<i4"), ("first", "<i4"), ("pad", "<i4")])
+                                         ("C", "<i4"), ("first", "<i4"), ("overwrite", "<i4")])
         blocks = 0
-        for i, (pg, pb, dg, db, N, C) in enumerate(key):
-            rec[i] = (pg, pb, dg, db, N, C, blocks, 0)
+        for i, (pg, pb, dg, db, N, C, ow) in enumerate(key):
+            rec[i] = (pg, pb, dg, db, N, C, blocks, ow)
             blocks += (C + 255) // 256
         table = torch.from_numpy(rec.view(np.uint8).copy()).to(dev)
         if len(_gn_tables) > 64:
@@ -314,7 +351,8 @@
         return
 
     def go():
-        _wgrad_launch(x, dy, N, H, W, cin, Ho, Wo, cout, ks, stride, out=slot, dbias=bslot)
+        _wgrad_launch(x, dy, N, H, W, cin, Ho, Wo, cout, ks, stride, out=slot, dbias=bslot,
+                      accumulate=_claim(weight, bias if bslot is not None else None))
         _grad_sink.ready(weight)
         if bslot is not None:
             _grad_sink.ready(bias)
@@ -552,7 +590,9 @@
     return _prof_wrap(name, flops, go)
 
 
-def _wgrad_launch(x, dy, N, H, W, Cin, Ho, Wo, Cout, ks, stride, out=None, dbias=None):
+def _wgrad_launch(x, dy, N, H, W, Cin, Ho, Wo, Cout, ks, stride, out=None, dbias=None, accumulate=None):
+    if accumulate is None:
+        accumulate = 0 if out is None else 1
     L = _lib.lib()
     splits = ctypes.c_int(0)
     wsb = ctypes.c_size_t(0)
@@ -575,18 +615,18 @@
         if _prof_shapes:
             name += " M=%d N=%d K=%d" % (M, Cout, K)
         _prof_wrap(name, 2.0 * M * Cout * K, go)
-    _lib.check(L.mdm_conv_wgrad_reduce(_p(ws), _p(dw), _p(dbias), _p(dy), M, Cin, Cout, ks, 0 if out is None else 1, _dt(x),
+    _lib.check(L.mdm_conv_wgrad_reduce(_p(ws), _p(dw), _p(dbias), _p(dy), M, Cin, Cout, ks, accumulate, _dt(x),
                                        _stream()), "mdm_conv_wgrad_reduce")
     return dw
 
 
-def _colsum_launch(x2d, M, C, out=None):
+def _colsum_launch(x2d, M, C, out=None, accumulate=None):
     L = _lib.lib()
     nb = ctypes.c_int(0)
     wsb = ctypes.c_size_t(0)
     _lib.check(L.mdm_colsum_plan(M, C, ctypes.byref(nb), ctypes.byref(wsb)), "mdm_colsum_plan")
     ws = _f32_ws(wsb.value, x2d.device)
-    acc = 0 if out is None else 1
+    acc = (0 if out is None else 1) if accumulate is None else accumulate
     if out is None:
         out = torch.empty(C, dtype=torch.float32, device=x2d.device)
     _lib.check(L.mdm_colsum(_p(x2d), _p(out), _p(ws), M, C, acc, _dt(x2d), _stream()), "mdm_colsum")
@@ -690,7 +730,7 @@
     if want_b:
         slot = None if cout_pad != cout else _slot(bias)
         if slot is not None:
-            _colsum_launch(dy, N * Ho * Wo, cout_pad, out=slot)
+            _colsum_launch(dy, N * Ho * Wo, cout_pad, out=slot, accumulate=_claim(bias))
             _grad_sink.ready(bias)
         else:
             db = _colsum_launch(dy, N * Ho * Wo, cout_pad)[:cout]
@@ -859,7 +899,8 @@
                            "mdm_conv_wgrad_reduce")
                 dwo = slot if sunk else torch.empty(weight.shape, dtype=torch.float32, device=x.device)
                 dbo = (bslot if sunk else torch.empty(cout, dtype=torch.float32, device=x.device)) if want_b else None
-                _lib.check(L.mdm_upconv_wfold(_p(dwb), _p(dwo), _p(db4), _p(dbo), cout, cin, 1 if sunk else 0, _stream()), "mdm_upconv_wfold")
+                acc = _claim(weight, bias if want_b else None) if sunk else 0
+                _lib.check(L.mdm_upconv_wfold(_p(dwb), _p(dwo), _p(db4), _p(dbo), cout, cin, acc, _stream()), "mdm_upconv_wfold")
                 if sunk:
                     _grad_sink.ready(weight)
                     if want_b:
@@ -1408,6 +1449,8 @@
     dfilm = torch.empty_like(film) if film is not None else None
     ws = _gn_ws(N, HW, C, groups, x.device)
     mode = 2 if (deferred or rows) else (1 if sunk else 0)
+    if mode == 1:
+        _adding(gamma, beta)
     npass = 3.0 + (dres is not None) + (dres2 is not None)
     _prof_wrap("group_norm bwd (HW=%d)" % HW, npass * x.numel() * x.element_size(), lambda: _lib.check(
         _lib.lib().mdm_gn_bwd(_p(dy), _p(x), _p(g32), _p(b32), _p(film), _p(stats), _p(coef), _p(dres), _p(dres2), _p(dx), _p(dgamma),
@@ -1561,6 +1604,8 @@
         dgamma = sg if sunk else torch.empty(D, dtype=torch.float32, device=x.device)
         dbeta = sb if sunk else torch.empty(D, dtype=torch.float32, device=x.device)
         ws = torch.empty(((R + 63) // 64) * D * 2, dtype=torch.float32, device=x.device)
+        if sunk:
+            _adding(gamma, beta)
         _lib.check(_lib.lib().mdm_ln_bwd(_p(dy), _p(x), _p(g32), _p(stats), _p(dx), _p(dgamma), _p(dbeta), _p(ws), R, D,
                                          1 if sunk else 0, _dt(x), _stream()), "mdm_ln_bwd")
         if sunk:
@@ -1645,7 +1690,8 @@
 
             def go(xs2=xs2, dy2=dy2, dws=dws, dbs=dbs, idx=idx, sunk=sunk, cout=cout):
                 _prof_wrap("conv_wgrad grouped x%d M=%d N=%d K=%d" % (len(idx), R, cout, D), 2.0 * len(idx) * R * cout * D,
-                           lambda: wgrad_grouped(xs2, dy2, dws, dbs))
+                           lambda: wgrad_grouped(xs2, dy2, dws, dbs,
+                                                 overwrite=[_claim(ws[l], bs[l]) == 0 for l in idx] if sunk else None))
                 if sunk:
                     for l in idx:
                         _grad_sink.ready(ws[l])
@@ -1668,6 +1714,8 @@
             dgs = [torch.empty(D, dtype=torch.float32, device=cond.device) for _ in range(L)]
             dbs_ = [torch.empty(D, dtype=torch.float32, device=cond.device) for _ in range(L)]
         dcond = torch.empty_like(cond)
+        if nsunk:
+            _adding(*lnw, *lnb)
         _lib.check(lib.mdm_ln_multi_bwd(_ptr_array(dcn), _p(cond), _ptr_array(g32), _p(stats), _p(dcond), _ptr_array(dgs),
                                         _ptr_array(dbs_), L, R, D, 1 if nsunk else 0, _dt(cond), _stream()), "mdm_ln_multi_bwd")
         if nsunk:
@@ -1736,7 +1784,8 @@
 
             def go(xs2=xs2, dy2=dy2, dws=dws, dbs=dbs, idx=idx, sunk=sunk, cout=cout):
                 _prof_wrap("conv_wgrad grouped x%d M=%d N=%d K=%d" % (len(idx), R, cout, D), 2.0 * len(idx) * R * cout * D,
-                           lambda: wgrad_grouped(xs2, dy2, dws, dbs))
+                           lambda: wgrad_grouped(xs2, dy2, dws, dbs,
+                                                 overwrite=[_claim(ws[l], bs[l]) == 0 for l in idx] if sunk else None))
                 if sunk:
                     for l in idx:
                         _grad_sink.ready(ws[l])
@@ -2711,11 +2760,12 @@
 def adamw_ema_step(p, g, m, v, ema, gnorm_sq, lr, beta1, beta2, eps, weight_decay, step, clip, ema_decay, zero_grad=True,
                    step_dev=None):
     _require_gpu(p)
-    nbytes = 4.0 * p.numel() * ((4 if ema is None else 5) + (3 if ema is None else 4) + (1 if zero_grad else 0))
+    zero_grad = int(zero_grad)
+    nbytes = 4.0 * p.numel() * ((4 if ema is None else 5) + (3 if ema is None else 4) + (1 if zero_grad == 1 else 0))
     _prof_wrap("adamw_ema_step", nbytes, lambda: _lib.check(
         _lib.lib().mdm_adamw_ema_step(_p(p), _p(g), _p(m), _p(v), _p(ema), _p(gnorm_sq), p.numel(), float(lr), float(beta1),
                                       float(beta2), float(eps), float(weight_decay), int(step), _p(step_dev), float(clip), float(ema_decay),
-                                      1 if zero_grad else 0, _stream()),
+                                      zero_grad, _stream()),
         "mdm_adamw_ema_step",
     ), kind="hbm")
     invalidate_packed_weights()
diff --git a/ml-mdm_amd/mdm_hip/trainer.py b/ml-mdm_amd/mdm_hip/trainer.py
--- a/ml-mdm_amd/mdm_hip/trainer.py
+++ b/ml-mdm_amd/mdm_hip/trainer.py
@@ -52,6 +52,7 @@
         ops.flush_wgrad_queue()
         self.reducer.mark("bw1")
         ops.join_side_stream()
+        self.reducer.settle()
         self.reducer.finish()
 
     def post_scalar(self, name, value):
@@ -83,7 +84,8 @@
             self.reducer.flat[:1].add_(loss.detach().float().reshape(1) * 0.0)
         ops.sumsq(self.reducer.flat, out=self.gnorm_sq, step_counter=self.step_dev)
         ops.adamw_ema_step(self.flat_p, self.reducer.flat, self.m, self.v, self.flat_ema, self.gnorm_sq, lr, betas[0], betas[1],
-                           eps, weight_decay, 0, clip_norm, ema_decay, zero_grad=True, step_dev=self.step_dev)
+                           eps, weight_decay, 0, clip_norm, ema_decay, zero_grad=2, step_dev=self.step_dev)
+        self.reducer.step_done()
         ops.repack_all(dtype)
 
 
```
